# mightypirate1/DRL-Tetris

Hardware: AMD Instinct MI355X
Metric: env-steps/sec at 64k parallel 20x10 boards (higher is better)
Workload: dtype u32

## Files before the change

### drl-tetris_amd/csrc/tetris_aql.h

```cpp
#pragma once
#include <hsa/hsa.h>
#include <hsa/hsa_ext_amd.h>
#include <dlfcn.h>
#include <atomic>
#include <immintrin.h>

namespace aql {

struct Kernel { uint64_t object = 0; uint32_t kernarg = 0, group = 0, priv = 0; bool ok = false; };

struct Queues {
    hsa_queue_t* q[CHAIN_STREAMS] = {};
    char* kernarg[CHAIN_STREAMS] = {};
    uint32_t slot_bytes = 0;
    std::atomic<uint64_t> issued[CHAIN_STREAMS];
    hsa_signal_t gate[CHAIN_STREAMS][2] = {};
    hsa_signal_t done[CHAIN_STREAMS] = {};
    hsa_signal_t first{};
    bool ok = false;
    uint32_t xcd_base[CHAIN_STREAMS] = {};
    bool affine_ok = false, calibrated = false;
};
struct Device {
    int hip_device = -1;
    bool tried = false, ok = false;
    hsa_agent_t gpu{}, cpu{};
    hsa_amd_memory_pool_t dev_pool{};
    uint64_t ts_freq = 0;
    std::vector<hsa_executable_t> exes;
    Kernel chain1, chain1_affine, duo, duo_affine, blocker, xcc_probe;
    std::vector<std::vector<char>> images;
    Queues qs;
    std::string why;
};

constexpr int SLOTS = 4096;
constexpr uint32_t QUEUE_PACKETS = 1024;

static std::mutex g_mutex;
static std::vector<Device*> g_devices;

struct FindCtx { Device* d; uint32_t want_bdf; uint32_t want_domain; bool found_gpu = false, found_cpu = false; };

static hsa_status_t on_agent(hsa_agent_t a, void* p) {
    FindCtx* c = (FindCtx*)p;
    hsa_device_type_t t;
    if (hsa_agent_get_info(a, HSA_AGENT_INFO_DEVICE, &t) != HSA_STATUS_SUCCESS) return HSA_STATUS_SUCCESS;
    if (t == HSA_DEVICE_TYPE_CPU && !c->found_cpu) { c->d->cpu = a; c->found_cpu = true; }
    if (t == HSA_DEVICE_TYPE_GPU && !c->found_gpu) {
        uint32_t bdf = 0, domain = 0;
        (void)hsa_agent_get_info(a, (hsa_agent_info_t)HSA_AMD_AGENT_INFO_BDFID, &bdf);
        (void)hsa_agent_get_info(a, (hsa_agent_info_t)HSA_AMD_AGENT_INFO_DOMAIN, &domain);
        if ((bdf & 0xFFFFu) == c->want_bdf && domain == c->want_domain) { c->d->gpu = a; c->found_gpu = true; }
    }
    return HSA_STATUS_SUCCESS;
}
static hsa_status_t on_gpu_pool(hsa_amd_memory_pool_t p, void* out) {
    Device* d = (Device*)out;
    hsa_amd_segment_t seg;
    uint32_t flags = 0;
    bool alloc = false;
    if (hsa_amd_memory_pool_get_info(p, HSA_AMD_MEMORY_POOL_INFO_SEGMENT, &seg) != HSA_STATUS_SUCCESS || seg != HSA_AMD_SEGMENT_GLOBAL) return HSA_STATUS_SUCCESS;
    (void)hsa_amd_memory_pool_get_info(p, HSA_AMD_MEMORY_POOL_INFO_GLOBAL_FLAGS, &flags);
    (void)hsa_amd_memory_pool_get_info(p, HSA_AMD_MEMORY_POOL_INFO_RUNTIME_ALLOC_ALLOWED, &alloc);
    if (alloc && (flags & HSA_AMD_MEMORY_POOL_GLOBAL_FLAG_COARSE_GRAINED) && d->dev_pool.handle == 0) d->dev_pool = p;
    return HSA_STATUS_SUCCESS;
}
struct SymCtx { Device* d; };
static hsa_status_t on_symbol(hsa_executable_t, hsa_agent_t, hsa_executable_symbol_t s, void* p) {
    Device* d = ((SymCtx*)p)->d;
    hsa_symbol_kind_t kind;
    if (hsa_executable_symbol_get_info(s, HSA_EXECUTABLE_SYMBOL_INFO_TYPE, &kind) != HSA_STATUS_SUCCESS || kind != HSA_SYMBOL_KIND_KERNEL) return HSA_STATUS_SUCCESS;
    uint32_t len = 0;
    (void)hsa_executable_symbol_get_info(s, HSA_EXECUTABLE_SYMBOL_INFO_NAME_LENGTH, &len);
    std::string name(len, '\0');
    (void)hsa_executable_symbol_get_info(s, HSA_EXECUTABLE_SYMBOL_INFO_NAME, &name[0]);
    Kernel* k = nullptr;
    if (name.rfind("_Z7k_chainILi1EEvN2te5KArgsE", 0) == 0) k = &d->chain1;
    else if (name.rfind("_Z5k_duoILi6ELb1ELb0EEvN2te5KArgsE", 0) == 0) k = &d->duo;
    else if (name.rfind("_Z9k_blockerPKjy", 0) == 0) k = &d->blocker;
    else if (name.rfind("_Z14k_chain_affineILi1EEvN2te5KArgsE", 0) == 0) k = &d->chain1_affine;
    else if (name.rfind("tetris_k_xcc_probe", 0) == 0) k = &d->xcc_probe;
    else if (name.rfind("_Z12k_duo_affineN2te5KArgsE", 0) == 0) k = &d->duo_affine;
    if (!k) return HSA_STATUS_SUCCESS;
    bool ok = hsa_executable_symbol_get_info(s, HSA_EXECUTABLE_SYMBOL_INFO_KERNEL_OBJECT, &k->object) == HSA_STATUS_SUCCESS;
    ok = ok && hsa_executable_symbol_get_info(s, HSA_EXECUTABLE_SYMBOL_INFO_KERNEL_KERNARG_SEGMENT_SIZE, &k->kernarg) == HSA_STATUS_SUCCESS;
    ok = ok && hsa_executable_symbol_get_info(s, HSA_EXECUTABLE_SYMBOL_INFO_KERNEL_GROUP_SEGMENT_SIZE, &k->group) == HSA_STATUS_SUCCESS;
    ok = ok && hsa_executable_symbol_get_info(s, HSA_EXECUTABLE_SYMBOL_INFO_KERNEL_PRIVATE_SEGMENT_SIZE, &k->priv) == HSA_STATUS_SUCCESS;
    k->ok = ok && k->object != 0;
    return HSA_STATUS_SUCCESS;
}

static bool own_code_objects(std::vector<std::vector<char>>& out, std::string& why) {
    Dl_info info;
    if (!dladdr((const void*)&own_code_objects, &info) || !info.dli_fname) { why = "dladdr failed"; return false; }
    FILE* f = fopen(info.dli_fname, "rb");
    if (!f) { why = std::string("cannot read ") + info.dli_fname; return false; }
    std::vector<char> file;
    fseek(f, 0, SEEK_END);
    const long len = ftell(f);
    fseek(f, 0, SEEK_SET);
    if (len <= 0) { fclose(f); why = "empty library file"; return false; }
    file.resize((size_t)len);
    const size_t got = fread(file.data(), 1, file.size(), f);
    fclose(f);
    if (got != file.size()) { why = "short read of the library file"; return false; }
    static const char magic[] = "__CLANG_OFFLOAD_BUNDLE__";
    const size_t mlen = sizeof magic - 1;
    for (size_t at = 0; at + mlen + 8 <= file.size(); ) {
        const void* hit = memmem(file.data() + at, file.size() - at, magic, mlen);
        if (!hit) break;
        const size_t base = (size_t)((const char*)hit - file.data());
        at = base + mlen;
        uint64_t n = 0;
        memcpy(&n, file.data() + base + mlen, 8);
        size_t o = base + mlen + 8;
        if (n == 0 || n > 64) continue;
        for (uint64_t e = 0; e < n; e++) {
            if (o + 24 > file.size()) break;
            uint64_t off, size, idlen;
            memcpy(&off, file.data() + o, 8); memcpy(&size, file.data() + o + 8, 8); memcpy(&idlen, file.data() + o + 16, 8);
            o += 24;
            if (idlen > 256 || o + idlen > file.size()) break;
            const std::string id(file.data() + o, (size_t)idlen);
            o += (size_t)idlen;
            if (id.find("amdgcn-amd-amdhsa") != std::string::npos && id.find("gfx950") != std::string::npos && size > 0 &&
                base + off + size <= file.size())
                out.emplace_back(file.data() + base + off, file.data() + base + off + size);
        }
    }
    if (out.empty()) { why = "no gfx950 code object found in the library's fat binary"; return false; }
    return true;
}

static Device* device_for(int hip_device) {
    std::lock_guard<std::mutex> lock(g_mutex);
    for (Device* d : g_devices) if (d->hip_device == hip_device) return d;
    Device* d = new Device();
    d->hip_device = hip_device;
    d->tried = true;
    g_devices.push_back(d);
    auto bad = [&](const std::string& w) { d->why = w; d->ok = false; return d; };
    {
        const char* tools[] = {getenv("ROCP_TOOL_LIBRARIES"), getenv("HSA_TOOLS_LIB"), getenv("LD_PRELOAD")};
        for (const char* t : tools)
            if (t && (strstr(t, "rocprofiler") || strstr(t, "roctracer") || strstr(t, "rocprof")) && !getenv("TETRIS_DIRECT_UNDER_TOOLS"))
                return bad("a profiling tool intercepts the HSA queues");
    }
    hipDeviceProp_t prop;
    if (hipGetDeviceProperties(&prop, hip_device) != hipSuccess) return bad("hipGetDeviceProperties failed");
    if (hsa_init() != HSA_STATUS_SUCCESS) return bad("hsa_init failed");
    FindCtx fc{d, (uint32_t)(((uint32_t)prop.pciBusID << 8) | ((uint32_t)prop.pciDeviceID << 3)), (uint32_t)prop.pciDomainID};
    (void)hsa_iterate_agents(on_agent, &fc);
    if (!fc.found_gpu || !fc.found_cpu) return bad("no HSA agent with the HIP device's PCI address");
    (void)hsa_amd_agent_iterate_memory_pools(d->gpu, on_gpu_pool, d);
    if (d->dev_pool.handle == 0) return bad("no coarse-grained device memory pool");
    (void)hsa_system_get_info(HSA_SYSTEM_INFO_TIMESTAMP_FREQUENCY, &d->ts_freq);
    if (!d->ts_freq) return bad("no timestamp frequency");
    std::string why;
    if (!own_code_objects(d->images, why)) return bad(why);
    for (auto& img : d->images) {
        hsa_code_object_reader_t reader;
        hsa_executable_t exe;
        if (hsa_code_object_reader_create_from_memory(img.data(), img.size(), &reader) != HSA_STATUS_SUCCESS) continue;
        if (hsa_executable_create_alt(HSA_PROFILE_FULL, HSA_DEFAULT_FLOAT_ROUNDING_MODE_DEFAULT, nullptr, &exe) != HSA_STATUS_SUCCESS) continue;
        if (hsa_executable_load_agent_code_object(exe, d->gpu, reader, nullptr, nullptr) != HSA_STATUS_SUCCESS ||
            hsa_executable_freeze(exe, nullptr) != HSA_STATUS_SUCCESS) { (void)hsa_executable_destroy(exe); continue; }
        d->exes.push_back(exe);
        SymCtx sc{d};
        (void)hsa_executable_iterate_agent_symbols(exe, d->gpu, on_symbol, &sc);
    }
    if (!d->chain1.ok || !d->duo.ok) return bad("the chained kernels were not found in the loaded code objects");
    if (d->chain1.priv || d->duo.priv) return bad("the chained kernels use scratch memory");
    const uint32_t explicit_bytes = (uint32_t)((sizeof(KArgs) + 7) & ~(size_t)7);
    if (d->chain1.kernarg < explicit_bytes || d->duo.kernarg < explicit_bytes || d->chain1.kernarg > 1024 || d->duo.kernarg > 1024)
        return bad("unexpected kernel-argument segment size");
    d->ok = true;
    return d;
}

static void destroy_queues(Queues& qs) {
    for (int k = 0; k < CHAIN_STREAMS; k++) {
        if (qs.q[k]) (void)hsa_queue_destroy(qs.q[k]);
        if (qs.kernarg[k]) (void)hsa_amd_memory_pool_free(qs.kernarg[k]);
        for (int s = 0; s < 2; s++) if (qs.gate[k][s].handle) (void)hsa_signal_destroy(qs.gate[k][s]);
        if (qs.done[k].handle) (void)hsa_signal_destroy(qs.done[k]);
    }
    if (qs.first.handle) (void)hsa_signal_destroy(qs.first);
    for (int k = 0; k < CHAIN_STREAMS; k++) { qs.q[k] = nullptr; qs.kernarg[k] = nullptr; qs.done[k] = hsa_signal_t{}; qs.gate[k][0] = qs.gate[k][1] = hsa_signal_t{}; }
    qs.first = hsa_signal_t{}; qs.ok = false; qs.affine_ok = false; qs.calibrated = false;
}

static bool make_queues(Device* d, std::string& why) {
    std::lock_guard<std::mutex> lock(g_mutex);
    Queues& qs = d->qs;
    const int depth = CHAIN_STREAMS;
    if (qs.ok) return true;
    for (int k = 0; k < CHAIN_STREAMS; k++) qs.issued[k].store(0);
    qs.slot_bytes = ((std::max(d->chain1.kernarg, d->duo.kernarg) + 63u) & ~63u) + 64u;
    for (int k = 0; k < depth; k++) {
        if (hsa_queue_create(d->gpu, QUEUE_PACKETS, HSA_QUEUE_TYPE_MULTI, nullptr, nullptr, UINT32_MAX, UINT32_MAX, &qs.q[k]) != HSA_STATUS_SUCCESS) { why = "hsa_queue_create failed"; destroy_queues(qs); return false; }
        (void)hsa_amd_profiling_set_profiler_enabled(qs.q[k], 1);
        if (hsa_amd_memory_pool_allocate(d->dev_pool, (size_t)SLOTS * qs.slot_bytes + 4096, 0, (void**)&qs.kernarg[k]) != HSA_STATUS_SUCCESS ||
            hsa_amd_agents_allow_access(1, &d->cpu, nullptr, qs.kernarg[k]) != HSA_STATUS_SUCCESS) { why = "no host-visible device memory for the kernel arguments"; destroy_queues(qs); return false; }
        for (int s = 0; s < 2; s++)
            if (hsa_signal_create(0, 0, nullptr, &qs.gate[k][s]) != HSA_STATUS_SUCCESS) { why = "hsa_signal_create failed"; destroy_queues(qs); return false; }
        if (hsa_signal_create(0, 0, nullptr, &qs.done[k]) != HSA_STATUS_SUCCESS) { why = "hsa_signal_create failed"; destroy_queues(qs); return false; }
    }
    if (hsa_signal_create(0, 0, nullptr, &qs.first) != HSA_STATUS_SUCCESS) { why = "hsa_signal_create failed"; destroy_queues(qs); return false; }
    qs.ok = true;
    return true;
}

static void fill_hidden(char* slot, uint32_t explicit_bytes, uint32_t slot_bytes, uint32_t blocks, uint32_t group) {
    char* h = slot + explicit_bytes;
    const uint32_t room = slot_bytes - explicit_bytes;
    if (room < 72) return;
    const uint32_t bc[3] = {blocks, 1u, 1u};
    const uint16_t gs[3] = {(uint16_t)group, 1, 1};
    const uint16_t dims = 1;
    memcpy(h + 0, bc, 12);
    memcpy(h + 12, gs, 6);
    memcpy(h + 64, &dims, 2);
}

static inline bool wait_signal(hsa_signal_t s) {
    for (int round = 0; round < 4000; round++)
        if (hsa_signal_wait_scacquire(s, HSA_SIGNAL_CONDITION_LT, 1, 2000000, HSA_WAIT_STATE_ACTIVE) < 1) return true;
    return hsa_signal_wait_scacquire(s, HSA_SIGNAL_CONDITION_LT, 1, UINT64_MAX, HSA_WAIT_STATE_BLOCKED) < 1;
}

struct Pending {
    uint64_t written[CHAIN_STREAMS] = {}, rung[CHAIN_STREAMS] = {};
    bool wrote[CHAIN_STREAMS] = {};
    char* last_slot = nullptr;
};
static inline void ring(Queues& qs, Pending& pd) {
    if (pd.last_slot) { _mm_sfence(); (void)*(volatile uint32_t*)pd.last_slot; pd.last_slot = nullptr; }
    for (int k = 0; k < CHAIN_STREAMS; k++)
        if (pd.wrote[k] && pd.written[k] != pd.rung[k]) {
            hsa_signal_store_screlease(qs.q[k]->doorbell_signal, (hsa_signal_value_t)(pd.written[k] - 1));
            pd.rung[k] = pd.written[k];
        }
}
static inline char* claim_packet(Queues& qs, Pending& pd, int k) {
    hsa_queue_t* q = qs.q[k];
    const uint64_t idx = hsa_queue_add_write_index_relaxed(q, 1);
    while (idx - hsa_queue_load_read_index_scacquire(q) >= q->size) ring(qs, pd);
    pd.written[k] = idx + 1; pd.wrote[k] = true;
    return (char*)q->base_address + (idx & (q->size - 1)) * 64;
}
static inline void write_dispatch(Queues& qs, Pending& pd, int k, const Kernel& kern, const void* args, size_t arg_bytes, uint32_t blocks,
                                  int acquire, int release, hsa_signal_t signal) {
    char* slot = qs.kernarg[k] + (size_t)(qs.issued[k].fetch_add(1) % SLOTS) * qs.slot_bytes;
    memcpy(slot, args, arg_bytes);
    fill_hidden(slot, (uint32_t)((arg_bytes + 7) & ~(size_t)7), qs.slot_bytes, blocks, 64);
    pd.last_slot = slot;
    char* p = claim_packet(qs, pd, k);
    hsa_kernel_dispatch_packet_t* d = (hsa_kernel_dispatch_packet_t*)p;
    d->setup = 1 << HSA_KERNEL_DISPATCH_PACKET_SETUP_DIMENSIONS;
    d->workgroup_size_x = 64; d->workgroup_size_y = 1; d->workgroup_size_z = 1; d->reserved0 = 0;
    d->grid_size_x = blocks * 64u; d->grid_size_y = 1; d->grid_size_z = 1;
    d->private_segment_size = kern.priv; d->group_segment_size = kern.group;
    d->kernel_object = kern.object; d->kernarg_address = slot; d->reserved2 = 0; d->completion_signal = signal;
    const uint16_t header = (uint16_t)((HSA_PACKET_TYPE_KERNEL_DISPATCH << HSA_PACKET_HEADER_TYPE) | (1 << HSA_PACKET_HEADER_BARRIER) |
                                       (acquire << HSA_PACKET_HEADER_SCACQUIRE_FENCE_SCOPE) | (release << HSA_PACKET_HEADER_SCRELEASE_FENCE_SCOPE));
    __atomic_store_n((uint16_t*)p, header, __ATOMIC_RELEASE);
}
static inline void write_barrier(Queues& qs, Pending& pd, int k, hsa_signal_t signal, int scope = HSA_FENCE_SCOPE_SYSTEM) {
    char* p = claim_packet(qs, pd, k);
    memset(p + 2, 0, 62);
    ((hsa_barrier_and_packet_t*)p)->completion_signal = signal;
    const uint16_t header = (uint16_t)((HSA_PACKET_TYPE_BARRIER_AND << HSA_PACKET_HEADER_TYPE) | (1 << HSA_PACKET_HEADER_BARRIER) |
                                       (scope << HSA_PACKET_HEADER_SCACQUIRE_FENCE_SCOPE) | (scope << HSA_PACKET_HEADER_SCRELEASE_FENCE_SCOPE));
    __atomic_store_n((uint16_t*)p, header, __ATOMIC_RELEASE);
}

static void calibrate_affine(Device* d) {
    std::lock_guard<std::mutex> lock(g_mutex);
    Queues& qs = d->qs;
    if (!qs.ok || qs.calibrated) return;
    qs.calibrated = true;
    { const char* e = getenv("TETRIS_AFFINE"); if (e && e[0] == '0') return; }
    if (!d->xcc_probe.ok || !d->chain1_affine.ok || d->xcc_probe.priv || d->chain1_affine.priv || (d->duo_affine.ok && d->duo_affine.priv)) return;
    constexpr uint32_t BLOCKS = 1024;
    const size_t words = (size_t)2 * CHAIN_STREAMS * BLOCKS;
    uint32_t* out = nullptr;
    if (hsa_amd_memory_pool_allocate(d->dev_pool, words * 4, 0, (void**)&out) != HSA_STATUS_SUCCESS) return;
    std::vector<uint32_t> host(words, 0xFFu);
    bool ok = hsa_memory_copy(out, host.data(), words * 4) == HSA_STATUS_SUCCESS;
    for (int rep = 0; rep < 2 && ok; rep++) {
        Pending pd;
        for (int k = 0; k < CHAIN_STREAMS; k++) {
            struct { uint32_t* out; } args = {out + ((size_t)rep * CHAIN_STREAMS + k) * BLOCKS};
            hsa_signal_store_relaxed(qs.done[k], 1);
            write_dispatch(qs, pd, k, d->xcc_probe, &args, sizeof args, BLOCKS, HSA_FENCE_SCOPE_SYSTEM, HSA_FENCE_SCOPE_SYSTEM, qs.done[k]);
        }
        ring(qs, pd);
        for (int k = 0; k < CHAIN_STREAMS; k++) ok = wait_signal(qs.done[k]) && ok;
    }
    ok = ok && hsa_memory_copy(host.data(), out, words * 4) == HSA_STATUS_SUCCESS;
    (void)hsa_amd_memory_pool_free(out);
    if (!ok) return;
    for (int k = 0; k < CHAIN_STREAMS; k++) {
        const uint32_t* a = &host[(size_t)k * BLOCKS];
        const uint32_t* b = &host[((size_t)CHAIN_STREAMS + k) * BLOCKS];
        if (a[0] > 7u || a[0] != b[0]) return;
        for (uint32_t i = 0; i < BLOCKS; i++)
            if (a[i] != ((a[0] + i) & 7u) || b[i] != a[i]) return;
        qs.xcd_base[k] = a[0];
    }
    qs.affine_ok = true;
}

static inline void quiesce(Queues& qs) {
    if (!qs.ok) return;
    Pending pd;
    for (int k = 0; k < CHAIN_STREAMS; k++)
        if (qs.q[k]) { hsa_signal_store_relaxed(qs.done[k], 1); write_barrier(qs, pd, k, qs.done[k]); }
    ring(qs, pd);
    for (int k = 0; k < CHAIN_STREAMS; k++)
        if (qs.q[k]) (void)wait_signal(qs.done[k]);
}

}
```

### drl-tetris_amd/csrc/tetris_engine.h

```cpp
#pragma once
#include "tetris_layout.h"
#include "tetris_tables.h"

#if defined(__clang__)
#define TE_UNROLL _Pragma("unroll")
#else
#define TE_UNROLL _Pragma("GCC unroll 8")
#endif

namespace te {

TE_HD int ctz32(uint32_t v) { return __builtin_ctz(v); }
TE_HD int clz32(uint32_t v) { return __builtin_clz(v); }
#if defined(__HIP_DEVICE_COMPILE__)
TE_HD uint32_t ld_stream(const uint32_t* p) { return __builtin_nontemporal_load(p); }
TE_HD void st_stream(uint32_t* p, uint32_t v) { __builtin_nontemporal_store(v, p); }
#else
TE_HD uint32_t ld_stream(const uint32_t* p) { return *p; }
TE_HD void st_stream(uint32_t* p, uint32_t v) { *p = v; }
#endif

#if defined(TE_PATH_COUNTERS) && !defined(__HIPCC__)
enum PathCounter { PC_KICK = 0, PC_KICK_2ND, PC_KICK_3RD, PC_KICK_FAILED, PC_KICK_DOWN, PC_DROP_EXACT, PC_RT_OFF_SPAWN,
                   PC_GARBAGE_ROW, PC_GARBAGE_LIFT2, PC_DEATH_GARBAGE, PC_DEATH_SPAWN, PC_TIMER_LOCK, PC_KEY_KICK, PC_KEY_KICK_FAILED,
                   PC_UNDO_SIMPLE, PC_UNDO_FULL, PC_UNDO_MISPREDICT, PC_NCOUNTERS };
extern unsigned long long te_path_count[PC_NCOUNTERS];
#define TE_COUNT(i) (te_path_count[i]++)
#else
#define TE_COUNT(i) do {} while (0)
#endif

enum MemMode : int { MEM_STREAM = 0, MEM_AGENT = 1, MEM_AFFINE = 2 };
#if defined(__HIP_DEVICE_COMPILE__)
TE_HD uint32_t ld_agent(const uint32_t* p) { return __hip_atomic_load(p, __ATOMIC_RELAXED, __HIP_MEMORY_SCOPE_AGENT); }
TE_HD void st_agent(uint32_t* p, uint32_t v) { __hip_atomic_store(p, v, __ATOMIC_RELAXED, __HIP_MEMORY_SCOPE_AGENT); }
#else
TE_HD uint32_t ld_agent(const uint32_t* p) { return *p; }
TE_HD void st_agent(uint32_t* p, uint32_t v) { *p = v; }
#endif
#if defined(__HIP_DEVICE_COMPILE__)
TE_HD __amdgpu_buffer_rsrc_t te_rsrc(const void* base) {
    return __builtin_amdgcn_make_buffer_rsrc(const_cast<void*>(base), (short)0, -1, 0x00020000);
}
constexpr int TE_AUX_NT = 2, TE_AUX_SC1 = 16;
TE_HD uint32_t ldw(const uint32_t* base, uint32_t o, size_t word_off, int mem = MEM_STREAM) {
    const __amdgpu_buffer_rsrc_t r = te_rsrc(base);
    if (mem == MEM_AGENT || mem == MEM_AFFINE) return __builtin_amdgcn_raw_buffer_load_b32(r, (int)o, (int)(uint32_t)(word_off * 4u), TE_AUX_SC1);
    return __builtin_amdgcn_raw_buffer_load_b32(r, (int)o, (int)(uint32_t)(word_off * 4u), TE_AUX_NT);
}
TE_HD void stw(uint32_t* base, uint32_t o, size_t word_off, uint32_t v, int mem = MEM_STREAM) {
    const __amdgpu_buffer_rsrc_t r = te_rsrc(base);
    if (mem == MEM_AGENT) __builtin_amdgcn_raw_buffer_store_b32(v, r, (int)o, (int)(uint32_t)(word_off * 4u), TE_AUX_SC1);
    else if (mem == MEM_AFFINE) __builtin_amdgcn_raw_buffer_store_b32(v, r, (int)o, (int)(uint32_t)(word_off * 4u), 0);
    else __builtin_amdgcn_raw_buffer_store_b32(v, r, (int)o, (int)(uint32_t)(word_off * 4u), TE_AUX_NT);
}
#else
TE_HD uint32_t ldw(const uint32_t* base, uint32_t o, size_t word_off, int mem = MEM_STREAM) {
    const uint32_t* p = (const uint32_t*)((const char*)(base + word_off) + o);
    return mem != MEM_STREAM ? ld_agent(p) : ld_stream(p);
}
TE_HD void stw(uint32_t* base, uint32_t o, size_t word_off, uint32_t v, int mem = MEM_STREAM) {
    uint32_t* p = (uint32_t*)((char*)(base + word_off) + o);
    if (mem != MEM_STREAM) st_agent(p, v); else st_stream(p, v);
}
#endif
#if defined(__HIP_DEVICE_COMPILE__)
TE_HD void add_word(uint32_t* p, uint32_t v) { (void)__hip_atomic_fetch_add(p, v, __ATOMIC_RELAXED, __HIP_MEMORY_SCOPE_AGENT); }
#else
TE_HD void add_word(uint32_t* p, uint32_t v) { *p += v; }
#endif
#if defined(__HIP_DEVICE_COMPILE__)
TE_HD uint32_t mul24(uint32_t a, uint32_t b) { return __umul24(a, b); }
#else
TE_HD uint32_t mul24(uint32_t a, uint32_t b) { return a * b; }
#endif
TE_HD int imin(int a, int b) { return a < b ? a : b; }
TE_HD int imax(int a, int b) { return a > b ? a : b; }
TE_HD uint32_t f2u(float f) { union { float f; uint32_t u; } v; v.f = f; return v.u; }
TE_HD float u2f(uint32_t u) { union { float f; uint32_t u; } v; v.u = u; return v.f; }

constexpr uint16_t SHAPE_ROWS[7][4] = {
    {0x2260, 0x0710, 0x3220, 0x4700}, {0x2230, 0x1700, 0x6220, 0x0740}, {0x2640, 0x0630, 0x1320, 0x6300},
    {0x2310, 0x3600, 0x4620, 0x0360}, {0x2222, 0x0f00, 0x4444, 0x00f0}, {0x0720, 0x2320, 0x2700, 0x2620},
    {0x0660, 0x0660, 0x0660, 0x0660},
};
TE_HD int spawn_rot(int kind) { return (int)((0x0977u >> (2 * (kind & 7))) & 3u); }
TE_HD int shape_value(int kind) { return (int)((0x06127534u >> (4 * (kind & 7))) & 15u); }

constexpr uint32_t make_shape(int kind, int rot) {
    uint32_t rows = SHAPE_ROWS[kind][rot];
    uint32_t nibs = 0;
    for (int gy = 0; gy < 4; gy++) {
        uint32_t rown = (rows >> (4 * (3 - gy))) & 0xF;
        for (int gx = 0; gx < 4; gx++)
            if ((rown >> gx) & 1) nibs |= 1u << (4 * gx + gy);
    }
    int minc = 3, maxc = 0;
    for (int gx = 0; gx < 4; gx++)
        if ((nibs >> (4 * gx)) & 0xF) { if (gx < minc) minc = gx; if (gx > maxc) maxc = gx; }
    return nibs | ((uint32_t)minc << 16) | ((uint32_t)maxc << 18);
}
constexpr uint32_t make_drop_word(uint32_t nibs) {
    uint32_t w = 0;
    for (int gx = 0; gx < 4; gx++) {
        uint32_t n = (nibs >> (4 * gx)) & 0xF;
        int bottom = -1;
        for (int gy = 0; gy < 4; gy++)
            if ((n >> gy) & 1) bottom = gy;
        w |= (uint32_t)(bottom < 0 ? 0x7F : 0x40 - (bottom + 1)) << (8 * gx);
    }
    return w;
}
constexpr int SHAPE_WORDS = 64;
struct ShapeTable { uint32_t s[SHAPE_WORDS]; };
constexpr ShapeTable make_shape_table() {
    ShapeTable t{};
    for (int k = 0; k < 7; k++)
        for (int r = 0; r < 4; r++) {
            t.s[k * 4 + r] = make_shape(k, r);
            t.s[32 + k * 4 + r] = make_drop_word(t.s[k * 4 + r] & 0xFFFFu);
        }
    for (int r = 0; r < 4; r++) { t.s[28 + r] = 0; t.s[60 + r] = 0x7F7F7F7Fu; }
    return t;
}
constexpr ShapeTable SHAPES = make_shape_table();

struct Ctx {
    const uint32_t* shapes;
    const uint8_t* table;
    const uint64_t* start;
    const double* combo_pow;
    uint32_t n_draws;
    uint32_t margin;
    int H;
    uint32_t floor_bits;
    bool tint;
    bool queue;
};

constexpr int ERR_FIFO = 1;
constexpr int ERR_STREAM = 2;

struct Raw8 { uint32_t lo, hi; };
struct Player {
    uint32_t col[NCOL];
    uint32_t tint[3][NCOL];
    int kind, rot, x, y, next;
    int dead, lock_armed, reward;
    int inc_count, combo_count, line_count, qlen;
    int q_overflow;
    int32_t time_ms, drop_delay, drop_time, speedup_time, lock_time;
    int32_t combo_start, combo_time, min_remaining;
    uint32_t combo_remaining;
    float incoming;
    uint32_t piece_draws, hole_draws;
    uint32_t pgroup;
    uint32_t lines_sent, lines_cleared, lines_blocked, max_combo, lines_seen, garbage_cleared;
    int32_t qcount[FIFO_CAP];
    int32_t qdelay[FIFO_CAP];
    int q_loaded;
    Raw8 pf_raw;
    int pf_ok;
};

struct ResetPrefetch { uint32_t seed16; uint64_t word; int ok; };

template <int P>
struct Game {
    Player pl[P];
    uint32_t seed16;
    int round_over, last_winner;
    uint32_t flags;
    uint32_t episode;
    uint32_t steps;
    uint32_t add_lines, add_sent;
    uint32_t status;
    uint32_t draw0, draw1;
};

TE_HD void load_player(const uint32_t* s, uint32_t o, size_t ws, Player& q, bool tint, bool queue = true, int mem = MEM_STREAM) {
    for (int c = 0; c < NCOL; c++) q.col[c] = ldw(s, o, (size_t)(W_COL0 + c) * ws, mem);
    if (tint)
        for (int k = 0; k < 3; k++)
            for (int c = 0; c < NCOL; c++) q.tint[k][c] = ldw(s, o, (size_t)(W_TINT0 + 10 * k + c) * ws, mem);
    uint32_t w = ldw(s, o, (size_t)W_PIECE * ws, mem);
    q.kind = w & 7; q.rot = (w >> 3) & 3; q.x = (int)((w >> 5) & 15) - 4; q.y = (w >> 9) & 31;
    q.next = (w >> 14) & 7; q.dead = (w >> 17) & 1; q.lock_armed = (w >> 18) & 1; q.reward = (w >> 19) & 255;
    w = ldw(s, o, (size_t)W_MISC * ws, mem);
    q.inc_count = w & 255; q.combo_count = (w >> 8) & 255; q.line_count = (w >> 16) & 255;
    q.qlen = (w >> 24) & 15; q.q_overflow = (w >> 28) & 3;
    if (!queue) { q.inc_count = 0; q.qlen = 0; q.q_overflow = 0; }
    q.time_ms = (int32_t)ldw(s, o, (size_t)W_TIME * ws, mem);
    w = ldw(s, o, (size_t)W_DROPCOMBO * ws, mem);
    q.drop_delay = w & 0xFFFF; q.combo_remaining = w >> 16;
    q.drop_time = (int32_t)ldw(s, o, (size_t)W_DROP_TIME * ws, mem);
    q.speedup_time = (int32_t)ldw(s, o, (size_t)W_SPEEDUP_TIME * ws, mem);
    q.lock_time = (int32_t)ldw(s, o, (size_t)W_LOCK_TIME * ws, mem);
    q.combo_start = (int32_t)ldw(s, o, (size_t)W_COMBO_START * ws, mem);
    q.combo_time = (int32_t)ldw(s, o, (size_t)W_COMBO_TIME * ws, mem);
    q.incoming = queue ? u2f(ldw(s, o, (size_t)W_INCOMING * ws, mem)) : 0.0f;
    q.min_remaining = queue ? (int32_t)ldw(s, o, (size_t)W_MIN_REMAINING * ws, mem) : 1000;
    q.piece_draws = ldw(s, o, (size_t)W_PIECE_DRAWS * ws, mem);
    q.hole_draws = queue ? ldw(s, o, (size_t)W_HOLE_DRAWS * ws, mem) : 0u;
    q.pgroup = ldw(s, o, (size_t)W_PIECE_GROUP * ws, mem);
    w = ldw(s, o, (size_t)W_STATS0 * ws, mem); q.lines_sent = w & 0xFFFF; q.lines_cleared = w >> 16;
    w = ldw(s, o, (size_t)W_STATS1 * ws, mem); q.lines_blocked = w & 0xFFFF; q.max_combo = w >> 16;
    w = ldw(s, o, (size_t)W_STATS2 * ws, mem); q.lines_seen = w & 0xFFFF; q.garbage_cleared = w >> 16;
    q.q_loaded = queue && q.qlen > 0;
    q.pf_ok = 0; q.pf_raw.lo = 0; q.pf_raw.hi = 0;
    if (queue)
        for (int i = 0; i < FIFO_CAP; i++) { q.qcount[i] = 0; q.qdelay[i] = 0; }
    if (q.q_loaded) {
        for (int i = 0; i < FIFO_CAP / 2; i++) {
            uint32_t cw = ldw(s, o, (size_t)(W_FIFO_COUNT0 + i) * ws, mem);
            q.qcount[2 * i] = (int16_t)(cw & 0xFFFF);
            q.qcount[2 * i + 1] = (int16_t)(cw >> 16);
        }
        for (int i = 0; i < FIFO_CAP; i++) q.qdelay[i] = (int32_t)ldw(s, o, (size_t)(W_FIFO_DELAY0 + i) * ws, mem);
    }
}

template <int P>
TE_HD void load_game_words(const Ref& gr, Game<P>& g, bool counters = false, int mem = MEM_STREAM) {
    uint32_t meta = ldw(gr.s, gr.o, (size_t)G_META * gr.ws, mem);
    g.seed16 = meta & 0xFFFFu;
    g.round_over = (meta >> 16) & 1;
    g.last_winner = (int)((meta >> 17) & 0xF) - 1;
    g.flags = (meta >> 21) & 7u;
    g.episode = ldw(gr.s, gr.o, (size_t)G_EPISODE * gr.ws, mem);
    g.steps = counters ? ldw(gr.s, gr.o, (size_t)G_STEPS * gr.ws, mem) : 0u;
    g.add_lines = 0; g.add_sent = 0;
    g.status = 0;
}

template <int P>
TE_HD void load_game(const Geo& geo_in, size_t slot, Game<P>& g, bool tint = false, bool queue = true, bool counters = false, int mem = MEM_STREAM) {
    Geo geo = geo_in;
    geo.P = P;
    load_game_words<P>(game_ref(geo, slot), g, counters, mem);
    TE_UNROLL
    for (int p = 0; p < P; p++) {
        const Ref r = board_ref(geo, p, slot);
        load_player(r.s, r.o, r.ws, g.pl[p], tint, queue, mem);
    }
}

TE_HD void store_player(uint32_t* s, uint32_t o, size_t ws, const Player& q, bool tint, bool queue = true, int mem = MEM_STREAM) {
    for (int c = 0; c < NCOL; c++) stw(s, o, (size_t)(W_COL0 + c) * ws, q.col[c], mem);
    if (tint)
        for (int k = 0; k < 3; k++)
            for (int c = 0; c < NCOL; c++) stw(s, o, (size_t)(W_TINT0 + 10 * k + c) * ws, q.tint[k][c], mem);
    stw(s, o, (size_t)W_PIECE * ws, (uint32_t)q.kind | ((uint32_t)q.rot << 3) | ((uint32_t)(q.x + 4) << 5) | ((uint32_t)q.y << 9) |
                              ((uint32_t)q.next << 14) | ((uint32_t)q.dead << 17) | ((uint32_t)q.lock_armed << 18) |
                              ((uint32_t)(q.reward & 255) << 19), mem);
    stw(s, o, (size_t)W_MISC * ws, (uint32_t)(q.inc_count & 255) | ((uint32_t)(q.combo_count & 255) << 8) |
                             ((uint32_t)(q.line_count & 255) << 16) | ((uint32_t)q.qlen << 24) | ((uint32_t)q.q_overflow << 28), mem);
    stw(s, o, (size_t)W_TIME * ws, (uint32_t)q.time_ms, mem);
    stw(s, o, (size_t)W_DROPCOMBO * ws, ((uint32_t)q.drop_delay & 0xFFFF) | (q.combo_remaining << 16), mem);
    stw(s, o, (size_t)W_DROP_TIME * ws, (uint32_t)q.drop_time, mem);
    stw(s, o, (size_t)W_SPEEDUP_TIME * ws, (uint32_t)q.speedup_time, mem);
    stw(s, o, (size_t)W_LOCK_TIME * ws, (uint32_t)q.lock_time, mem);
    stw(s, o, (size_t)W_COMBO_START * ws, (uint32_t)q.combo_start, mem);
    stw(s, o, (size_t)W_COMBO_TIME * ws, (uint32_t)q.combo_time, mem);
    if (queue) stw(s, o, (size_t)W_INCOMING * ws, f2u(q.incoming), mem);
    stw(s, o, (size_t)W_MIN_REMAINING * ws, (uint32_t)q.min_remaining, mem);
    stw(s, o, (size_t)W_PIECE_DRAWS * ws, q.piece_draws, mem);
    if (queue) stw(s, o, (size_t)W_HOLE_DRAWS * ws, q.hole_draws, mem);
    stw(s, o, (size_t)W_PIECE_GROUP * ws, q.pgroup, mem);
    stw(s, o, (size_t)W_STATS0 * ws, (q.lines_sent & 0xFFFF) | (q.lines_cleared << 16), mem);
    stw(s, o, (size_t)W_STATS1 * ws, (q.lines_blocked & 0xFFFF) | (q.max_combo << 16), mem);
    stw(s, o, (size_t)W_STATS2 * ws, (q.lines_seen & 0xFFFF) | (q.garbage_cleared << 16), mem);
    if (queue && (q.q_loaded || q.qlen > 0)) {
        for (int i = 0; i < FIFO_CAP / 2; i++)
            stw(s, o, (size_t)(W_FIFO_COUNT0 + i) * ws, ((uint32_t)q.qcount[2 * i] & 0xFFFF) | ((uint32_t)q.qcount[2 * i + 1] << 16), mem);
        for (int i = 0; i < FIFO_CAP; i++) stw(s, o, (size_t)(W_FIFO_DELAY0 + i) * ws, (uint32_t)q.qdelay[i], mem);
    }
}

template <int P>
TE_HD void store_game_words(const Ref& gr, const Game<P>& g, bool counters = false, int mem = MEM_STREAM) {
    stw(gr.s, gr.o, (size_t)G_META * gr.ws, g.seed16 | ((uint32_t)g.round_over << 16) | ((uint32_t)(g.last_winner + 1) << 17) | (g.flags << 21), mem);
    stw(gr.s, gr.o, (size_t)G_EPISODE * gr.ws, g.episode, mem);
    if (counters) stw(gr.s, gr.o, (size_t)G_STEPS * gr.ws, g.steps, mem);
    if (g.add_lines) add_word(&word_at(gr, G_LINES), g.add_lines);
    if (g.add_sent) add_word(&word_at(gr, G_SENT), g.add_sent);
}

template <int P>
TE_HD void store_game(const Geo& geo_in, size_t slot, const Game<P>& g, bool tint = false, bool queue = true, bool counters = false, int mem = MEM_STREAM) {
    Geo geo = geo_in;
    geo.P = P;
    store_game_words<P>(game_ref(geo, slot), g, counters, mem);
    TE_UNROLL
    for (int p = 0; p < P; p++) {
        const Ref r = board_ref(geo, p, slot);
        store_player(r.s, r.o, r.ws, g.pl[p], tint, queue, mem);
    }
}


TE_HD uint32_t shape_of(const Ctx& cx, int kind, int rot) { return cx.shapes[(kind << 2) | rot]; }

TE_HD uint64_t band_window(const Ctx& cx, const Player& q, int y) {
    uint32_t lo = 0xFFu, hi = 0xFFFF0000u;
    for (int c = 0; c < 6; c++) lo |= ((uint32_t)((int32_t)(q.col[c] | cx.floor_bits) >> y) & 0xFu) << (4 * c + 8);
    for (int c = 6; c < NCOL; c++) hi |= ((uint32_t)((int32_t)(q.col[c] | cx.floor_bits) >> y) & 0xFu) << (4 * (c - 6));
    return ((uint64_t)hi << 32) | lo;
}

TE_HD bool fits_band(uint64_t band, uint32_t shape, int x) {
    unsigned xs = (unsigned)(x + 2);
    if (xs > 12u) return false;
    return (((uint64_t)(shape & 0xFFFFu) << (4 * xs)) & band) == 0;
}

TE_HD bool fits_at(const Ctx& cx, const Player& q, uint32_t shape, int x, int y) {
    return fits_band(band_window(cx, q, y), shape, x);
}

TE_HD bool fits_spawn_col(const Ctx& cx, const Player& q, uint32_t shape, int y) {
    constexpr int X0 = (NCOL - 4) / 2;
    uint32_t hit = 0;
    TE_UNROLL
    for (int gx = 0; gx < 4; gx++) hit |= (q.col[X0 + gx] | cx.floor_bits) & (((shape >> (4 * gx)) & 0xFu) << y);
    return hit == 0;
}

TE_HD uint32_t col_at(const Player& q, int i) {
    uint32_t a0 = (i & 1) ? q.col[1] : q.col[0];
    uint32_t a1 = (i & 1) ? q.col[3] : q.col[2];
    uint32_t a2 = (i & 1) ? q.col[5] : q.col[4];
    uint32_t a3 = (i & 1) ? q.col[7] : q.col[6];
    uint32_t a4 = (i & 1) ? q.col[9] : q.col[8];
    uint32_t b0 = (i & 2) ? a1 : a0;
    uint32_t b1 = (i & 2) ? a3 : a2;
    uint32_t d0 = (i & 4) ? b1 : b0;
    return (i & 8) ? a4 : d0;
}

TE_HD int drop_distance(const Ctx& cx, const Player& q, uint32_t shape) {
    int dist = 64;
    for (int gx = 0; gx < 4; gx++) {
        uint32_t nib = (shape >> (4 * gx)) & 0xFu;
        if (nib) {
            int top = q.y + ctz32(nib);
            int bottom = q.y + (31 - clz32(nib));
            uint32_t below = (col_at(q, q.x + gx) | cx.floor_bits) >> (top + 1);
            int first = below ? ctz32(below) + top + 1 : 32;
            dist = imin(dist, imax(0, first - bottom - 1));
        }
    }
    return dist == 64 ? 0 : dist;
}

TE_HD int drop_distance_bytes(const Ctx& cx, const Player& q, uint32_t shape, uint32_t drop_word) {
    uint32_t d[NCOL];
    for (int c = 0; c < NCOL; c++) d[c] = (uint32_t)ctz32((q.col[c] | cx.floor_bits) >> q.y);
    const uint32_t w0 = (d[0] << 16) | (d[1] << 24);
    const uint32_t w1 = d[2] | (d[3] << 8) | (d[4] << 16) | (d[5] << 24);
    const uint32_t w2 = d[6] | (d[7] << 8) | (d[8] << 16) | (d[9] << 24);
    const unsigned xs = (unsigned)(q.x + 2);
    const bool hi2 = (xs & 8u) != 0, hi1 = (xs & 4u) != 0;
    const uint32_t lo = hi2 ? (hi1 ? 0u : w2) : (hi1 ? w1 : w0);
    const uint32_t hi = hi2 ? 0u : (hi1 ? w2 : w1);
#if defined(__HIP_DEVICE_COMPILE__)
    const uint32_t under = __builtin_amdgcn_alignbyte(hi, lo, xs & 3u);
#else
    const uint32_t under = (uint32_t)((((uint64_t)hi << 32) | lo) >> (8 * (xs & 3u)));
#endif
    const uint32_t sum = under + drop_word;
    const uint32_t b0 = sum & 0xFFu, b1 = (sum >> 8) & 0xFFu, b2 = (sum >> 16) & 0xFFu, b3 = sum >> 24;
    const uint32_t m01 = b0 < b1 ? b0 : b1, m23 = b2 < b3 ? b2 : b3;
    const uint32_t m = m01 < m23 ? m01 : m23;
    if (m - 0x40u > 0x3Eu) { TE_COUNT(PC_DROP_EXACT); return drop_distance(cx, q, shape); }
    return (int)(m - 0x40u);
}

TE_HD void stamp(const Ctx& cx, Player& q, uint32_t shape) {
    unsigned xs = (unsigned)(q.x + 2);
    if (xs > 12u) return;
    uint64_t placed = (uint64_t)(shape & 0xFFFFu) << (4 * xs);
    for (int c = 0; c < NCOL; c++) {
        const uint32_t cells = ((uint32_t)(placed >> (4 * c + 8)) & 0xFu) << q.y;
        q.col[c] |= cells;
        if (cx.tint)
            for (int k = 0; k < 3; k++) q.tint[k][c] = (q.tint[k][c] & ~cells) | (((q.kind >> k) & 1) ? cells : 0u);
    }
}

TE_HD int clear_rows(const Ctx& cx, Player& q) {
    uint32_t range = (~0u << q.y) & ~cx.floor_bits;
    int cleared = 0;
    for (;;) {
        uint32_t full = range;
        for (int c = 0; c < NCOL; c++) full &= q.col[c];
        if (!full) break;
        int r = 31 - clz32(full);
        uint32_t above = (1u << r) - 1u;
        uint32_t keep = ~((above << 1) | 1u);
        if (cx.tint) {
            uint32_t garbage = 0;
            for (int c = 0; c < NCOL; c++) garbage |= q.col[c] & q.tint[0][c] & q.tint[1][c] & q.tint[2][c];
            if ((garbage >> r) & 1u) q.garbage_cleared = (q.garbage_cleared + 1u) & 0xFFFFu;
            for (int k = 0; k < 3; k++)
                for (int c = 0; c < NCOL; c++) q.tint[k][c] = (q.tint[k][c] & keep) | ((q.tint[k][c] & above) << 1);
        }
        for (int c = 0; c < NCOL; c++) q.col[c] = (q.col[c] & keep) | ((q.col[c] & above) << 1);
        cleared++;
    }
    return cleared;
}

TE_HD uint32_t table_byte(const Ctx& cx, uint32_t seed16, uint32_t draw, uint32_t& status) {
    if (draw + cx.margin >= cx.n_draws) {
        status |= ST_NEED_EXTEND;
        if (draw >= cx.n_draws) { status |= ST_STREAM_EXHAUSTED; draw = cx.n_draws - 1; }
    }
    uint32_t chunk = draw / (uint32_t)CHUNK;
    uint32_t r = draw - mul24(chunk, (uint32_t)CHUNK);
    return cx.table[mul24((chunk << 16) + seed16, (uint32_t)CHUNK) + r];
}

TE_HD Raw8 table_group_raw(const Ctx& cx, uint32_t seed16, uint32_t draw, uint32_t& status) {
    if (draw + 8u + cx.margin >= cx.n_draws) {
        status |= ST_NEED_EXTEND;
        if (draw + 8u > cx.n_draws) { status |= ST_STREAM_EXHAUSTED; draw = cx.n_draws - 8u; }
    }
    uint32_t chunk = draw / (uint32_t)CHUNK;
    uint32_t r = draw - mul24(chunk, (uint32_t)CHUNK);
    const uint8_t* p = cx.table + (mul24((chunk << 16) + seed16, (uint32_t)CHUNK) + r);
    Raw8 v;
#if defined(__HIP_DEVICE_COMPILE__)
    const uint2 w = *reinterpret_cast<const uint2*>(p);
    v.lo = w.x; v.hi = w.y;
#else
    v.lo = 0; v.hi = 0;
    for (int k = 0; k < 4; k++) { v.lo |= (uint32_t)p[k] << (8 * k); v.hi |= (uint32_t)p[4 + k] << (8 * k); }
#endif
    return v;
}
TE_HD uint32_t pack_group(Raw8 v) {
    const uint32_t a = v.lo & 0x0F0F0F0Fu, b = v.hi & 0x0F0F0F0Fu;
    uint32_t lo = (a | (a >> 4)) & 0x00FF00FFu; lo = (lo | (lo >> 8)) & 0x0000FFFFu;
    uint32_t hi = (b | (b >> 4)) & 0x00FF00FFu; hi = (hi | (hi >> 8)) & 0x0000FFFFu;
    return lo | (hi << 16);
}

TE_HD void prefetch_next(const Ctx& cx, Player& q, uint32_t seed16, uint32_t& status) {
    q.pf_ok = 0;
    if ((q.piece_draws & 7u) == 7u) {
// ... 833 lines not shown
```

### drl-tetris_amd/csrc/tetris_hip.hip

```cpp
#include <hip/hip_runtime.h>
#include <hip/hip_ext.h>

#include <math.h>
#include <stdio.h>
#include <stdlib.h>
#include <string.h>

#include <algorithm>
#include <atomic>
#include <mutex>
#include <thread>
#include <new>
#include <chrono>
#include <string>
#include <vector>

#include "tetris_kernels.h"

using namespace te;


#include "tetris_game_kernel.h"

constexpr int CHAIN_LANES = 64;
constexpr int CHAIN_STREAMS = 3;
template <int P, bool AFFINE>
__device__ __forceinline__ void chain_body(const KArgs& a) {
    __shared__ __attribute__((aligned(16))) uint32_t s_shapes[SHAPE_WORDS];
    const int lane = threadIdx.x;
    if (a.steps < 0) { chain_census(a, lane == 0); return; }
    constexpr int CMEM = AFFINE ? MEM_AFFINE : MEM_AGENT;
    int wave = blockIdx.x;
    uint32_t xcc = 0;
    const auto report_xcc = [&]() { if (AFFINE && blockIdx.x == 0 && lane == 0) st_flag(a.status + F_XCC0 + (a.xcd_slot & 3u), 0x100u | xcc); };
    if (AFFINE) {
        asm volatile("s_getreg_b32 %0, hwreg(HW_REG_XCC_ID)" : "=s"(xcc));
        xcc &= 0xFu;
        if (xcc != ((a.xcd_base + blockIdx.x) & 7u)) {
            if (lane == 0) st_flag(a.status + F_PLACE, 1u);
            report_xcc();
            return;
        }
        wave = (int)((blockIdx.x & ~7u) | xcc);
        if (wave * CHAIN_LANES >= a.n) { report_xcc(); return; }
    }
    const int i = wave * CHAIN_LANES + lane;
    const bool active = lane < CHAIN_LANES && i < a.n;
    LaneCounters cnt = {0, 0, 0, 0};
    const uint32_t shape_word = d_shape_table.s[lane];
    Game<P> g;
    if (active) policy_draw(a, (uint32_t)i, a.first_step, g.draw0, g.draw1);
    const uint32_t d0 = g.draw0, d1 = g.draw1;
    int stride = a.n_stride;
    asm volatile("" : "+s"(stride));
    const uint32_t seen = chain_poll(a, (uint32_t)wave);
    if (seen == a.epoch - 1u) {
        Geo geo = geo_of(a);
        geo.stride = (size_t)stride;
        if (active) { load_game<P>(geo, (size_t)i, g, false, P > 1, true, CMEM); g.draw0 = d0; g.draw1 = d1; }
        s_shapes[lane] = shape_word;
        __builtin_amdgcn_wave_barrier();
        if (active) game_run<P, M_ROLLOUT, false, CMEM>(a, i, s_shapes, g, cnt);
        asm volatile("s_waitcnt vmcnt(0)" ::: "memory");
        if (lane == 0) {
            if (AFFINE) st_xcd(a.chain + (size_t)wave * CHAIN_STRIDE, a.epoch);
            else st_agent(a.chain + (size_t)wave * CHAIN_STRIDE, a.epoch);
        }
    } else if (!(seen & CHAIN_ABANDONED)) {
        chain_give_up(a, (uint32_t)wave, lane == 0);
    }
    report_xcc();
}
template <int P>
__global__ __launch_bounds__(64) void k_chain(KArgs a) { chain_body<P, false>(a); }
template <int P>
__global__ __launch_bounds__(64) void k_chain_affine(KArgs a) { chain_body<P, true>(a); }
template __global__ void k_chain_affine<1>(KArgs);
extern "C" __global__ void tetris_k_xcc_probe(uint32_t* out) {
    if (threadIdx.x == 0) {
        uint32_t xcc;
        asm volatile("s_getreg_b32 %0, hwreg(HW_REG_XCC_ID)" : "=s"(xcc));
        out[blockIdx.x] = xcc & 0xFu;
    }
}

__global__ void k_blocker(const uint32_t* go, unsigned long long ticks) {
    const unsigned long long t0 = __builtin_amdgcn_s_memrealtime();
    while (__builtin_amdgcn_s_memrealtime() - t0 < ticks) {
        if (go && __hip_atomic_load(go, __ATOMIC_RELAXED, __HIP_MEMORY_SCOPE_SYSTEM)) break;
        __builtin_amdgcn_s_sleep(32);
    }
}

__global__ void k_clock_probe(unsigned long long ticks, unsigned long long* out) {
    const unsigned long long r0 = __builtin_amdgcn_s_memrealtime(), c0 = __builtin_amdgcn_s_memtime();
    unsigned long long r1 = r0;
    while (r1 - r0 < ticks) { __builtin_amdgcn_s_sleep(4); r1 = __builtin_amdgcn_s_memrealtime(); }
    const unsigned long long c1 = __builtin_amdgcn_s_memtime();
    if (threadIdx.x == 0) { out[0] = c1 - c0; out[1] = r1 - r0; }
}

__global__ __launch_bounds__(256) void k_totals(Geo geo, unsigned long long* out ) {
    unsigned long long v[4] = {0, 0, 0, 0};
    for (int i = blockIdx.x * blockDim.x + threadIdx.x; i < (int)geo.n_games; i += gridDim.x * blockDim.x) {
        unsigned long long t[4];
        totals_of_game(geo, i, t);
        v[0] += t[0]; v[1] += t[1]; v[2] += t[2]; v[3] += t[3];
    }
    for (int k = 0; k < 4; k++) {
        for (int off = 32; off > 0; off >>= 1) v[k] += __shfl_down(v[k], off);
        if ((threadIdx.x & 63) == 0 && v[k]) atomicAdd(&out[k], v[k]);
    }
}

#define TE_OBS_BUILD(a, row, sl, i, COL, qx, qy, qnext, qkind, qinc, qcombo, qrem)                                              \
    do {                                                                                                                        \
        uint32_t col_[NCOL];                                                                                                    \
        TE_UNROLL                                                                                                               \
        for (int c = 0; c < NCOL; c++) col_[c] = COL(c);                                                                        \
        for (int yp = 0; yp < (a).H / 2; yp++) {                                                                                \
            uint32_t lo[NCOL], hi[NCOL];                                                   \
            TE_UNROLL                                                                                                           \
            for (int c = 0; c < NCOL; c++) { lo[c] = col_[c] & 1u; hi[c] = (col_[c] >> 1) & 1u; col_[c] >>= 2; }                \
            (row)[5 * yp + 0] = lo[0] | (lo[1] << 8) | (lo[2] << 16) | (lo[3] << 24);                                           \
            (row)[5 * yp + 1] = lo[4] | (lo[5] << 8) | (lo[6] << 16) | (lo[7] << 24);                                           \
            (row)[5 * yp + 2] = lo[8] | (lo[9] << 8) | (hi[0] << 16) | (hi[1] << 24);                                           \
            (row)[5 * yp + 3] = hi[2] | (hi[3] << 8) | (hi[4] << 16) | (hi[5] << 24);                                           \
            (row)[5 * yp + 4] = hi[6] | (hi[7] << 8) | (hi[8] << 16) | (hi[9] << 24);                                           \
        }                                                                                                                       \
                             \
        const uint32_t x_ = (uint32_t)(qx) & 0xFFu, y_ = (uint32_t)(qy) & 31u, next_ = (uint32_t)(qnext) & 7u;                  \
        uint32_t t_ = (((uint32_t)(qrem) & 0xFFFFu) + 50u) & 0xFFFFu;  \
        if (t_ > 25000u) t_ = 25000u;                                                                                           \
        uint32_t* v_ = (uint32_t*)((a).obs_vector + ((size_t)(sl) * (a).n + (i)) * 12);                                         \
        const uint64_t hot_ = next_ < 7u ? (1ull << (8 * next_)) : 0ull;                                       \
        v_[0] = x_ | (y_ << 8) | (((uint32_t)(qinc) & 255u) << 16) | ((t_ / 100u) << 24);                                       \
        v_[1] = ((uint32_t)(qcombo) & 255u) | ((uint32_t)(hot_ & 0xFFFFFFu) << 8);                                              \
        v_[2] = (uint32_t)(hot_ >> 24);                                                                                         \
        (a).obs_piece[(size_t)(sl) * (a).n + (i)] = (uint8_t)((uint32_t)(qkind) & 7u);                                          \
    } while (0)
__device__ __forceinline__ void obs_build(const KArgs& a, uint32_t* row, int sl, int i, uint32_t c0, uint32_t c1, uint32_t c2, uint32_t c3, uint32_t c4,
                                          uint32_t c5, uint32_t c6, uint32_t c7, uint32_t c8, uint32_t c9, int qx, int qy, int qnext, int qkind,
                                          int inc_count, int combo_count, uint32_t combo_remaining) {
    const uint32_t cols[NCOL] = {c0, c1, c2, c3, c4, c5, c6, c7, c8, c9};
#define TE_OBS_COL(c) cols[c]
    TE_OBS_BUILD(a, row, sl, i, TE_OBS_COL, qx, qy, qnext, qkind, inc_count, combo_count, combo_remaining);
#undef TE_OBS_COL
}
__device__ __forceinline__ void obs_stream(const KArgs& a, const uint32_t* rows, int sl, int first, int nb, int lane) {
    const int nw = a.H * NCOL / 4;
    uint32_t* dst = (uint32_t*)(a.obs_visual + ((size_t)sl * a.n + first) * (size_t)(a.H * NCOL));
    const uint32_t words = (uint32_t)nb * (uint32_t)nw;
    typedef uint32_t u32x4 __attribute__((ext_vector_type(4)));
    if (((((uintptr_t)dst) | ((uintptr_t)rows)) & 15u) == 0) {
        const uint32_t whole = words & ~3u;
        for (uint32_t k = 4u * (uint32_t)lane; k < whole; k += 4u * 64u)
            __builtin_nontemporal_store(*reinterpret_cast<const u32x4*>(rows + k), reinterpret_cast<u32x4*>(dst + k));
        if ((uint32_t)lane < words - whole) dst[whole + lane] = rows[whole + lane];
    } else
        for (uint32_t k = (uint32_t)lane; k < words; k += 64u) dst[k] = rows[k];
}

template <int P>
__device__ __forceinline__ void observe_emit(const KArgs& a, const Game<P>& g, int first, int lane, bool active, uint32_t* tile) {
    const int pitch = a.H * NCOL / 4, i = first + lane;
    const int nb = (a.n - first < 64) ? a.n - first : 64;
    const int me = active ? safe_player(a.next_player, i, P) : 0;
    TE_UNROLL
    for (int sl = 0; sl < P; sl++) {
        if (active) {
            const bool sel = P > 1 && (sl == 0 ? me == 1 : me == 0);
            const Player& q0 = g.pl[0];
            const Player& q1 = g.pl[P - 1];
            uint32_t* row = tile + (size_t)lane * pitch;
#define TE_OBS_COL(c) (sel ? q1.col[c] : q0.col[c])
            TE_OBS_BUILD(a, row, sl, i, TE_OBS_COL, sel ? q1.x : q0.x, sel ? q1.y : q0.y, sel ? q1.next : q0.next, sel ? q1.kind : q0.kind,
                         sel ? q1.inc_count : q0.inc_count, sel ? q1.combo_count : q0.combo_count, sel ? q1.combo_remaining : q0.combo_remaining);
#undef TE_OBS_COL
        }
        __syncthreads();
        obs_stream(a, tile, sl, first, nb, lane);
        __syncthreads();
    }
}

template <int MODE, bool CHAIN, bool OBS, bool AFFINE>
__device__ __forceinline__ void duo_body(const KArgs& a) {
    __shared__ __attribute__((aligned(16))) uint32_t s_shapes_all[4][SHAPE_WORDS];
    extern __shared__ __attribute__((aligned(16))) uint32_t s_duo_tile[];
    uint32_t* s_shapes = s_shapes_all[threadIdx.x >> 6];
    const uint32_t shape_word = d_shape_table.s[threadIdx.x & 63];
    const int lane = threadIdx.x & 63, side = lane >> 5;
    int wave = (blockIdx.x * blockDim.x + threadIdx.x) >> 6;
    constexpr bool ROLL = MODE == M_ROLLOUT, AUTO = MODE == M_STEP_RT_AUTO;
    constexpr int MEM = CHAIN ? (AFFINE ? MEM_AFFINE : MEM_AGENT) : MEM_STREAM;
    if (CHAIN && a.steps < 0) { chain_census(a, lane == 0); return; }
    uint32_t xcc = 0;
    const auto report_xcc = [&]() { if (AFFINE && blockIdx.x == 0 && lane == 0) st_flag(a.status + F_XCC0 + (a.xcd_slot & 3u), 0x100u | xcc); };
    if (AFFINE) {
        asm volatile("s_getreg_b32 %0, hwreg(HW_REG_XCC_ID)" : "=s"(xcc));
        xcc &= 0xFu;
        if (xcc != ((a.xcd_base + blockIdx.x) & 7u)) {
            if (lane == 0) st_flag(a.status + F_PLACE, 1u);
            report_xcc();
            return;
        }
        wave = (int)((blockIdx.x & ~7u) | xcc);
        if (wave * 32 >= a.n) { report_xcc(); return; }
    }
    const int gi = wave * 32 + (lane & 31);
    const bool active = gi < a.n;
    Geo geo = geo_of(a);
    geo.P = 2;
    const Ref gr = game_ref(geo, (size_t)gi);
    const Ref br = {geo.state, (uint32_t)((size_t)side * geo.stride + (size_t)gi) * 4u, 2 * geo.stride};
    Game<1> g;
    Player& q = g.pl[0];
    uint32_t pd0 = 0, pd1 = 0;
    if (CHAIN) {
        if (active) policy_draw(a, (uint32_t)gi, a.first_step, pd0, pd1);
        if (!chain_wait(a, (uint32_t)wave, lane == 0)) { report_xcc(); return; }
    }
    if (active) {
        load_game_words<1>(gr, g, ROLL, MEM);
        load_player(br.s, br.o, br.ws, q, false, true, MEM);
        if (CHAIN) { g.draw0 = pd0; g.draw1 = pd1; }
        else if (ROLL) policy_draw(a, (uint32_t)gi, a.first_step, g.draw0, g.draw1);
        else { g.draw0 = a.rot[gi]; g.draw1 = (uint32_t)a.trans[gi] | ((a.player ? (uint32_t)a.player[gi] : 0u) << 8); }
    }
    s_shapes[lane] = shape_word;
// ... 449 lines not shown
struct Tables {
    int device = -1;
    uint8_t map[8] = {0};
    int only_sz = 0;
    int refs = 0;
    uint32_t* d_mt = nullptr;
    float* d_w = nullptr;
    uint64_t* d_start = nullptr;
    double* d_pow = nullptr;
    uint8_t* d_table = nullptr;
    int n_chunks = 0, cap_chunks = 0;
    std::vector<uint8_t*> retired;
};
static const size_t CHUNK_BYTES = (size_t)65536 * CHUNK;
static std::mutex g_tab_mutex;
static std::vector<Tables*> g_tables;

static int tables_extend(Tables* t, hipStream_t stream) {
    if (t->n_chunks >= MAX_CHUNKS) return fail(TETRIS_E_STREAM, "RNG tables: MAX_CHUNKS reached");
    if (t->n_chunks == t->cap_chunks) {
        int cap = t->cap_chunks ? t->cap_chunks * 2 : 2;
        if (cap > MAX_CHUNKS) cap = MAX_CHUNKS;
        uint8_t* d = nullptr;
        HIP_TRY(hipMalloc((void**)&d, CHUNK_BYTES * cap));
        if (t->n_chunks) HIP_TRY(hipMemcpyAsync(d, t->d_table, CHUNK_BYTES * t->n_chunks, hipMemcpyDeviceToDevice, stream));
        if (t->d_table) t->retired.push_back(t->d_table);
        t->d_table = d;
        t->cap_chunks = cap;
    }
    MapArg m;
    memcpy(m.m, t->map, 8);
    hipLaunchKernelGGL(k_gen_chunk, dim3(256), dim3(256), 0, stream, t->d_mt, t->d_w, t->d_table + CHUNK_BYTES * t->n_chunks,
                       t->d_start, t->n_chunks, m, t->only_sz);
    HIP_TRY(hipGetLastError());
    HIP_TRY(hipStreamSynchronize(stream));
    t->n_chunks++;
    return TETRIS_OK;
}

static void tables_free(Tables* t) {
    (void)hipFree(t->d_mt); (void)hipFree(t->d_w); (void)hipFree(t->d_start); (void)hipFree(t->d_pow);
    (void)hipFree(t->d_table);
    for (uint8_t* c : t->retired) (void)hipFree(c);
    delete t;
}

static int tables_build(Tables* t, hipStream_t stream);

static int tables_acquire(Tables** out, int device, const uint8_t map[7], hipStream_t stream) {
    std::lock_guard<std::mutex> lock(g_tab_mutex);
    for (Tables* t : g_tables)
        if (t->device == device && memcmp(t->map, map, 7) == 0) { t->refs++; *out = t; return TETRIS_OK; }
    Tables* t = new (std::nothrow) Tables();
    if (!t) return fail(TETRIS_E_HIP, "out of host memory");
    t->device = device;
    memcpy(t->map, map, 7);
    t->only_sz = 1;
    for (int i = 0; i < 7; i++) if (map[i] != 2 && map[i] != 3) t->only_sz = 0;
    int rc = tables_build(t, stream);
    if (rc) { std::string keep = g_err; tables_free(t); return fail(rc, keep); }
    t->refs = 1;
    g_tables.push_back(t);
    *out = t;
    return TETRIS_OK;
}

static int tables_build(Tables* t, hipStream_t stream) {
    HIP_TRY(hipMalloc((void**)&t->d_mt, (size_t)624 * 65536 * 4));
    HIP_TRY(hipMalloc((void**)&t->d_w, (size_t)7 * 65536 * 4));
    HIP_TRY(hipMalloc((void**)&t->d_start, 65536 * sizeof(uint64_t)));
    HIP_TRY(hipMalloc((void**)&t->d_pow, 256 * sizeof(double)));
    double powtab[256];
    for (int c = 0; c < 256; c++) powtab[c] = pow((double)c, 1.4 + (double)c * 0.01);
    HIP_TRY(hipMemcpyAsync(t->d_pow, powtab, sizeof powtab, hipMemcpyHostToDevice, stream));
    hipLaunchKernelGGL(k_gen_seed, dim3(256), dim3(256), 0, stream, t->d_mt);
    HIP_TRY(hipGetLastError());
    HIP_TRY(hipStreamSynchronize(stream));
    for (int c = 0; c < 2; c++) {
        int rc = tables_extend(t, stream);
        if (rc) return rc;
    }
    return TETRIS_OK;
}

static void tables_release(Tables* t) {
    std::lock_guard<std::mutex> lock(g_tab_mutex);
    if (--t->refs > 0) return;
    for (size_t i = 0; i < g_tables.size(); i++)
        if (g_tables[i] == t) { g_tables.erase(g_tables.begin() + i); break; }
    tables_free(t);
}

struct Stage {
    void* h = nullptr;
    void* d = nullptr;
    size_t cap = 0;
    int ensure(size_t bytes) {
        if (bytes <= cap) return TETRIS_OK;
        size_t want = bytes < 4096 ? 4096 : bytes + bytes / 2;
        if (h) (void)hipHostFree(h);
        if (d) (void)hipFree(d);
        h = d = nullptr; cap = 0;
        HIP_TRY(hipHostMalloc(&h, want, hipHostMallocDefault));
        HIP_TRY(hipMalloc(&d, want));
        cap = want;
        return TETRIS_OK;
    }
    void release() {
        if (h) (void)hipHostFree(h);
        if (d) (void)hipFree(d);
        h = d = nullptr; cap = 0;
    }
};
constexpr int STAGES = 6;

constexpr int GATE_GROUP = 120;
#include "tetris_aql.h"

struct RolloutCall {
    uint32_t epoch0 = 0;
    uint64_t first_step = 0;
    int steps_per_launch = 0;
    uint32_t policy_seed = 0;
    int ms = 0;
    int launches = 0;
    bool chained = false;
};

struct tetris_batch {
    int device = 0, N = 0, P = 0, H = 0;
    int stride = 0;
    hipStream_t stream = nullptr;
    hipEvent_t ev0 = nullptr, ev1 = nullptr;
    uint32_t* d_state = nullptr;
    uint32_t* d_gstate = nullptr;
    uint32_t* flags = nullptr;
    unsigned long long* d_counters = nullptr;
    unsigned long long* h_counters = nullptr;
    Tables* tab = nullptr;
    uint32_t margin = 2 * (2 * GATE_GROUP + 2) + 16;
    uint32_t game_offset = 0;
    int split = 0, side = 0;
    int tint = 0, nw = NWORDS;
    int use_duo = 1;
    uint32_t* d_shadow = nullptr;
    hipStream_t own_stream = nullptr;
    hipStream_t chain_stream[CHAIN_STREAMS] = {};
    hipEvent_t chain_ev[CHAIN_STREAMS + 1] = {};
    hipEvent_t worker_gate_ev[CHAIN_STREAMS][2] = {};
    uint32_t* d_chain = nullptr;
    uint32_t chain_epoch = 0;
    int use_chain = 1;
    int use_graph = 0;
    long long chain_capacity = -1;
    int chain_depth = 0;
    bool chain_pending = false;
    uint32_t chain_spin_limit = CHAIN_SPIN_LIMIT;
    RolloutCall chain_call;
    bool chain_fell_back = false;
    uint32_t* h_chain = nullptr;
    hipStream_t stall_stream = nullptr;
    int direct_min = 16;
    bool last_direct = false;
    bool direct_used = false;
    int use_affine = 1;
    bool last_affine = false;
    uint32_t xcd_skew = 0;
    int affine_failures = 0;
    bool home_async = false;
    bool busy = true;
    hipEvent_t gate_ev[2] = {nullptr, nullptr};
    int gate_count = 0;
    int gate_slot = 0;
    int gate_pending[2] = {0, 0};
    Stage stage[STAGES];
    Stage recover_idx;
    uint8_t* d_plan_slabs = nullptr;
    size_t plan_slab_cap = 0;
    int32_t* d_iota = nullptr;
    uint32_t* d_plan_status = nullptr;
    int32_t* d_policy_scores = nullptr;
};

static Geo geo_of_batch(tetris_batch* b) {
    Geo g = {b->d_state, b->d_gstate, (size_t)b->N, b->P, b->nw, (size_t)b->stride};
    return g;
}

static KArgs base_args(tetris_batch* b, int n, const int32_t* d_idx) {
    KArgs a;
    memset(&a, 0, sizeof a);
    a.state = b->d_state; a.gstate = b->d_gstate; a.status = b->flags;
    {
        std::lock_guard<std::mutex> lock(g_tab_mutex);
        a.table = b->tab->d_table;
        a.n_draws = (uint32_t)b->tab->n_chunks * CHUNK;
    }
    a.start = b->tab->d_start; a.combo_pow = b->tab->d_pow; a.margin = b->margin;
    a.H = b->H; a.n_games = b->N; a.n_stride = b->stride; a.n_players = b->P; a.nw = b->nw; a.n = n; a.idx = d_idx; a.game_offset = b->game_offset;
    return a;
}

template <int MODE>
static int launch_game(tetris_batch* b, const KArgs& a) {
    dim3 grid((unsigned)((a.n + 255) / 256)), block(256);
    if constexpr (MODE == M_ROLLOUT || MODE == M_STEP_RT || MODE == M_STEP_RT_AUTO) {
        if (b->P == 2 && !b->tint && !a.idx && b->use_duo && (MODE != M_ROLLOUT || a.steps == 1)) {
            hipLaunchKernelGGL((k_duo<MODE>), dim3((unsigned)((a.n + 127) / 128)), block, 0, b->stream, a);
            HIP_TRY(hipGetLastError());
            return TETRIS_OK;
        }
    }
    const bool here = with_shape<1, 2>(b->P, b->tint != 0, [&](auto P, auto TINT) {
        hipLaunchKernelGGL((k_game<P(), MODE, TINT()>), grid, block, 0, b->stream, a);
    });
    if (!here && tetris_launch_game_multi(b->P, b->tint, MODE, grid, block, b->stream, a)) return fail(TETRIS_E_ARG, "no kernel for this player count / mode");
    HIP_TRY(hipGetLastError());
    return TETRIS_OK;
}

static int chain_lanes(const tetris_batch* b) { return b->P == 1 ? CHAIN_LANES : 32; }
static uint32_t chain_waves(const tetris_batch* b) { return (uint32_t)((b->N + chain_lanes(b) - 1) / chain_lanes(b)); }

static const void* chain_kernel(tetris_batch* b, long long* waves) {
    *waves = chain_waves(b);
    return b->P == 1 ? (const void*)k_chain<1> : (const void*)k_duo<M_ROLLOUT, true>;
}
static hipError_t launch_chain_kernel(tetris_batch* b, uint32_t blocks, hipStream_t st, const KArgs& a, hipEvent_t start = nullptr,
                                      hipEvent_t stop = nullptr) {
    if (b->P == 1) hipExtLaunchKernelGGL((k_chain<1>), dim3(blocks), dim3(64), 0, st, start, stop, 0, a);
    else hipExtLaunchKernelGGL((k_duo<M_ROLLOUT, true>), dim3(blocks), dim3(64), 0, st, start, stop, 0, a);
    return hipGetLastError();
}
static bool chain_census_ok(tetris_batch* b, long long waves) {
    uint32_t* d = nullptr;
    if (hipMalloc((void**)&d, 2 * CHAIN_STRIDE * sizeof(uint32_t)) != hipSuccess) return false;
    bool ok = false;
    uint32_t h[2] = {0, 1};
    KArgs a;
    memset(&a, 0, sizeof a);
    a.steps = -1; a.chain = d; a.epoch = (uint32_t)waves; a.chain_spin_limit = 4000;
    if (hipMemsetAsync(d, 0, 2 * CHAIN_STRIDE * sizeof(uint32_t), b->own_stream) == hipSuccess) {
        if (launch_chain_kernel(b, (uint32_t)waves, b->own_stream, a) == hipSuccess && hipMemcpyAsync(&h[0], d, 4, hipMemcpyDeviceToHost, b->own_stream) == hipSuccess &&
            hipMemcpyAsync(&h[1], d + CHAIN_STRIDE, 4, hipMemcpyDeviceToHost, b->own_stream) == hipSuccess &&
            hipStreamSynchronize(b->own_stream) == hipSuccess)
            ok = h[0] == (uint32_t)waves && h[1] == 0;
    }
    (void)hipFree(d);
    return ok;
}

static bool chain_fits(tetris_batch* b) {
    long long waves = 0;
    const void* fn = chain_kernel(b, &waves);
    static const int cap = [] { const char* e = getenv("TETRIS_CHAIN_DEPTH"); const int v = e ? atoi(e) : CHAIN_STREAMS; return v < 1 ? 1 : (v > CHAIN_STREAMS ? CHAIN_STREAMS : v); }();
    if (b->chain_capacity < 0) {
        int per_cu = 0, cus = 0;
        if (hipOccupancyMaxActiveBlocksPerMultiprocessor(&per_cu, fn, 64, 0) != hipSuccess) per_cu = 0;
        if (hipDeviceGetAttribute(&cus, hipDeviceAttributeMultiprocessorCount, b->device) != hipSuccess) cus = 0;
        b->chain_capacity = per_cu > 1 ? (long long)(per_cu - 1) * cus : 0;
        const long long full = (long long)per_cu * cus;
        int want = 0;
        for (int d = cap; d >= 2 && !want; d--)
            if (d * waves <= full) want = d;
        if (want && want * waves > b->chain_capacity && b->stream == b->own_stream && chain_census_ok(b, want * waves)) b->chain_capacity = want * waves;
    }
    b->chain_depth = 0;
    for (int d = cap; d >= 1 && !b->chain_depth; d--)
        if (d * waves <= b->chain_capacity) b->chain_depth = d;
    return b->chain_depth >= (cap == 1 ? 1 : 2);
}

static int service_flags(tetris_batch* b) {
    volatile uint32_t* f = b->flags;
    const uint32_t want = f[F_EXTEND];
    if (want) {
        std::lock_guard<std::mutex> lock(g_tab_mutex);
        if (want >= (uint32_t)b->tab->n_chunks * CHUNK && b->tab->n_chunks < MAX_CHUNKS) {
            int rc = tables_extend(b->tab, b->stream);
            if (rc) return rc;
            b->busy = true;
        }
        f[F_EXTEND] = 0;
    }
    return TETRIS_OK;
}

static hipError_t poll_event(hipEvent_t e, int spins) {
    hipError_t qe = hipErrorNotReady;
    for (int spin = 0; spin < spins && qe == hipErrorNotReady; spin++) qe = hipEventQuery(e);
    return qe == hipErrorNotReady ? hipEventSynchronize(e) : qe;
}

static int gate_launch(tetris_batch* b, int group) {
    if (b->gate_count >= group) {
        const int k = b->gate_slot;
        if (b->gate_pending[k]) {
            HIP_TRY(poll_event(b->gate_ev[k], 2000000));
            b->gate_pending[k] = 0;
        }
        HIP_TRY(hipEventRecord(b->gate_ev[k], b->stream));
        b->gate_pending[k] = 1;
        b->gate_slot = k ^ 1;
        b->gate_count = 0;
    }
    b->gate_count++;
    {
        bool on_chain = false;
        for (hipStream_t st : b->chain_stream) on_chain |= b->stream == st;
        if (!on_chain) b->home_async = true;
    }
    return service_flags(b);
}

static hipError_t drain_stream(hipStream_t st) {
    for (int spin = 0; spin < 20000; spin++) {
        const hipError_t e = hipStreamQuery(st);
        if (e != hipErrorNotReady) return e;
    }
    return hipStreamSynchronize(st);
}

static int finish_call(tetris_batch* b, bool drained = false) {
    if (!b->busy && !b->chain_pending && b->stream == b->own_stream) {
        int rc0 = service_flags(b);
        if (rc0) return rc0;
        if (!b->busy) return TETRIS_OK;
    }
    if (b->chain_pending && !drained)
        for (int k = 0; k < CHAIN_STREAMS; k++) HIP_TRY(drain_stream(b->chain_stream[k]));
    b->chain_pending = false;
    if (!drained) HIP_TRY(drain_stream(b->stream));
    b->home_async = false;
    b->busy = false;
    b->gate_count = 0; b->gate_pending[0] = b->gate_pending[1] = 0;
    volatile uint32_t* f = b->flags;
    int rc = TETRIS_OK;
    const bool misplaced = f[F_PLACE] != 0;
    if (misplaced) {
        const int keep_chain = b->use_chain;
        const bool keep_fell_back = b->chain_fell_back;
        f[F_PLACE] = 0;
        if ((rc = chain_recover(b))) return rc;
        b->use_chain = keep_chain; b->chain_fell_back = keep_fell_back;
        if (++b->affine_failures >= 3) b->use_affine = 0;
    }
    if (f[F_CHAIN] && (rc = chain_recover(b))) return rc;
    if ((rc = service_flags(b))) return rc;
    if (f[F_BADARG]) {
        f[F_BADARG] = 0;
        return fail(TETRIS_E_ARG, "output capacity exceeded (max_lists / max_keys too small)");
    }
    return TETRIS_OK;
}

static int check_batch(tetris_batch* b, bool enqueues = true) {
    if (!b) return fail(TETRIS_E_ARG, "null batch");
    HIP_TRY(hipSetDevice(b->device));
    if (enqueues) b->busy = true;
    return TETRIS_OK;
}

struct HostCall {
    tetris_batch* const b;
    const int32_t* d_idx = nullptr;
    int used = 0, n_out = 0;
    struct Out { const Stage* s; size_t bytes; void* dst; } outs[STAGES];

    int take(size_t bytes, Stage** s) {
        if (used >= STAGES) return fail(TETRIS_E_ARG, "internal: a call takes more than STAGES staging buffers");
        *s = &b->stage[used++];
        return (*s)->ensure(bytes + 16);
    }
    int send(const Stage* s, size_t bytes) {
        b->busy = true;
        HIP_TRY(hipMemcpyAsync(s->d, s->h, bytes, hipMemcpyHostToDevice, b->stream));
        return TETRIS_OK;
    }
    template <class T> int in(const T* src, size_t count, const T** d) {
        *d = nullptr;
        if (!src) { used++; return TETRIS_OK; }
        Stage* s;
        int rc = take(count * sizeof(T), &s);
        if (rc) return rc;
        memcpy(s->h, src, count * sizeof(T));
        *d = (const T*)s->d;
        return send(s, count * sizeof(T));
    }
    int idx(const int32_t* idx, int n) {
        if (n < 0 || (!idx && n > b->N)) return fail(TETRIS_E_ARG, "n out of range");
        for (int i = 0; idx && i < n; i++)
            if (idx[i] < 0 || idx[i] >= b->N) return fail(TETRIS_E_ARG, "game index out of range");
        return in(idx, (size_t)n, &d_idx);
    }
    template <class T> int out(void* dst, size_t count, T** d, const T** h = nullptr) {
        Stage* s;
        int rc = take(count * sizeof(T), &s);
        if (rc) return rc;
        outs[n_out++] = {s, count * sizeof(T), dst};
        *d = (T*)s->d;
        if (h) *h = (const T*)s->h;
        return TETRIS_OK;
    }
    int finish() {
        for (int k = 0; k < n_out; k++) {
            b->busy = true;
            HIP_TRY(hipMemcpyAsync(outs[k].s->h, outs[k].s->d, outs[k].bytes, hipMemcpyDeviceToHost, b->stream));
        }
        int rc = finish_call(b);
        if (rc) return rc;
        for (int k = 0; k < n_out; k++)
            if (outs[k].dst) memcpy(outs[k].dst, outs[k].s->h, outs[k].bytes);
        return TETRIS_OK;
    }
};

static int check_players(const tetris_batch* b, const uint8_t* player, int n) {
    for (int i = 0; player && i < n; i++)
        if (player[i] >= b->P) return fail(TETRIS_E_ARG, "player index out of range");
    return TETRIS_OK;
}

// ... 738 lines not shown
        uint8_t *d_cnt, *d_len, *d_key;
        if ((rc = io.idx(h_idx, m)) || (rc = io.in(player ? player + g0 : nullptr, (size_t)m, &d_player)) ||
            (rc = io.out(nullptr, lanes, &d_cnt, &hc)) || (rc = io.out(nullptr, lanes * L, &d_len, &hl)) ||
            (rc = io.out(nullptr, lanes * L * max_keys, &d_key, &hk))) return rc;
        dim3 grid((unsigned)((lanes + 63) / 64)), block(64);
        with_value<1, 4>(b->P, [&](auto P) {
            hipLaunchKernelGGL(k_actions<P()>, grid, block, 0, b->stream, geo_of_batch(b), m, io.d_idx, d_player, b->H, d_cnt, d_len, d_key,
                               PLAN_LANE_LISTS, max_keys, b->flags);
        });
        if (hipGetLastError() != hipSuccess) return fail(TETRIS_E_HIP, "k_actions launch failed");
        if ((rc = io.finish())) return rc;
        for (int i = 0; i < m; i++) {
            int total = 0;
            bool over = false;
            for (int xi = 0; xi < 10; xi++)
                for (int r = 0; r < 4; r++) {
                    const size_t lane = (size_t)i * 40 + r * 10 + xi;
                    for (int k = 0; k < hc[lane]; k++) {
                        if (total >= max_lists) { over = true; break; }
                        const int len = hl[lane * L + k];
                        lens[(size_t)(g0 + i) * max_lists + total] = (uint8_t)len;
                        memcpy(keys + ((size_t)(g0 + i) * max_lists + total) * max_keys, hk + (lane * L + k) * max_keys, (size_t)len);
                        total++;
                    }
                }
            count[g0 + i] = total;
            if (over) return fail(TETRIS_E_ARG, "more than max_lists key lists for one game");
        }
    }
    return TETRIS_OK;
}

static const int PLAN_CHUNK = 4096;

static int plan_check(tetris_batch* b, const char* what) {
    if (b->split) return fail(TETRIS_E_ARG, std::string(what) + " is not available on split batches");
    return TETRIS_OK;
}

static PlanArgs plan_args(tetris_batch* b, const uint8_t* d_player, const int32_t* d_count, const uint8_t* d_lens, const uint8_t* d_keys,
                          int max_lists, int max_keys, int ms) {
    PlanArgs pa;
    memset(&pa, 0, sizeof pa);
    pa.a = base_args(b, b->N, nullptr);
    pa.a.ms = ms;
    pa.player = d_player; pa.count = d_count; pa.lens = d_lens; pa.keys = d_keys;
    pa.max_lists = max_lists; pa.max_keys = max_keys;
    return pa;
}

static int launch_plan_kernel(tetris_batch* b, int which, dim3 grid, const PlanArgs& pa, int fin) {
    const bool here = with_shape<1, 2>(b->P, b->tint != 0, [&](auto P, auto TINT) { launch_plan<P(), TINT()>(which, grid, b->stream, pa, fin); });
    if (!here && tetris_launch_plan_multi(b->P, b->tint, which, grid, b->stream, pa, fin)) return fail(TETRIS_E_ARG, "no planning kernel for this player count");
    HIP_TRY(hipGetLastError());
    return TETRIS_OK;
}

int tetris_action_lists_dev(tetris_batch* b, const uint8_t* d_player, int max_lists, int max_keys, int flags, int32_t* d_count,
                            uint8_t* d_lens, uint8_t* d_keys) {
    int rc = check_batch(b);
    if (rc) return rc;
    if ((rc = plan_check(b, "tetris_action_lists_dev"))) return rc;
    if (!d_count || !d_lens || !d_keys) return fail(TETRIS_E_ARG, "count/lens/keys are NULL");
    if (max_lists < 1 || max_keys < 1 || max_keys > 254) return fail(TETRIS_E_ARG, "max_lists >= 1, 1 <= max_keys <= 254");
    if (flags & ~TETRIS_LISTS_KEEP_NULL) return fail(TETRIS_E_ARG, "unknown flag");
    const int chunk = b->N < PLAN_CHUNK ? b->N : PLAN_CHUNK;
    const int KS = max_keys + 1;
    const size_t lanes = (size_t)chunk * 40;
    const size_t need = lanes + lanes * PLAN_LANE_LISTS + lanes * PLAN_LANE_LISTS * KS;
    if (!b->d_iota) {
        std::vector<int32_t> iota((size_t)b->N);
        for (int i = 0; i < b->N; i++) iota[i] = i;
        HIP_TRY(hipMalloc((void**)&b->d_iota, (size_t)b->N * 4));
        HIP_TRY(hipMemcpy(b->d_iota, iota.data(), (size_t)b->N * 4, hipMemcpyHostToDevice));
        HIP_TRY(hipMalloc((void**)&b->d_plan_status, NFLAGS * 4));
    }
    if (need > b->plan_slab_cap) {
        if (b->d_plan_slabs) { HIP_TRY(hipStreamSynchronize(b->stream)); (void)hipFree(b->d_plan_slabs); }
        b->d_plan_slabs = nullptr; b->plan_slab_cap = 0;
        HIP_TRY(hipMalloc((void**)&b->d_plan_slabs, need));
        b->plan_slab_cap = need;
    }
    if ((rc = gate_launch(b, GATE_GROUP))) return rc;
    uint8_t* s_cnt = b->d_plan_slabs;
    uint8_t* s_len = s_cnt + lanes;
    uint8_t* s_key = s_len + lanes * PLAN_LANE_LISTS;
    const Geo geo = geo_of_batch(b);
    for (int g0 = 0; g0 < b->N; g0 += chunk) {
        const int m = b->N - g0 < chunk ? b->N - g0 : chunk;
        const int32_t* d_idx = b->d_iota + g0;
        const uint8_t* pl = d_player ? d_player + g0 : nullptr;
        const dim3 grid((unsigned)(((size_t)m * 40 + 63) / 64)), block(64);
        with_value<1, 4>(b->P, [&](auto P) {
            hipLaunchKernelGGL(k_actions<P()>, grid, block, 0, b->stream, geo, m, d_idx, pl, b->H, s_cnt, s_len, s_key, PLAN_LANE_LISTS, KS, b->d_plan_status);
        });
        HIP_TRY(hipGetLastError());
        hipLaunchKernelGGL(k_plan_lists, dim3((unsigned)m), block, 0, b->stream, s_cnt, s_len, s_key, KS, g0, max_lists, max_keys,
                           (flags & TETRIS_LISTS_KEEP_NULL) ? 1 : 0, d_count, d_lens, d_keys, b->flags);
        HIP_TRY(hipGetLastError());
    }
    return TETRIS_OK;
}

int tetris_simulate_lists_dev(tetris_batch* b, const uint8_t* d_player, const int32_t* d_count, const uint8_t* d_lens, const uint8_t* d_keys,
                              int max_lists, int max_keys, int ms, int flags, uint32_t* d_cols, uint8_t* d_done, uint8_t* d_lines,
                              uint8_t* d_dead) {
    int rc = check_batch(b);
    if (rc) return rc;
    if ((rc = plan_check(b, "tetris_simulate_lists_dev"))) return rc;
    if (!d_count || !d_lens || !d_keys || !d_cols) return fail(TETRIS_E_ARG, "count/lens/keys/cols are NULL");
    if (max_lists < 1 || max_lists > 65535 || max_keys < 1 || max_keys > 255) return fail(TETRIS_E_ARG, "1 <= max_lists <= 65535, 1 <= max_keys <= 255");
    if (flags & ~TETRIS_SIM_FINALIZE) return fail(TETRIS_E_ARG, "unknown flag");
    if ((rc = gate_launch(b, GATE_GROUP))) return rc;
    PlanArgs pa = plan_args(b, d_player, d_count, d_lens, d_keys, max_lists, max_keys, ms);
    pa.cols = d_cols;
    const int fin = (flags & TETRIS_SIM_FINALIZE) ? 1 : 0;
    if (fin) { pa.a.done = d_done; pa.a.lines = d_lines; pa.a.dead = d_dead; }
    return launch_plan_kernel(b, 0, dim3((unsigned)((b->N + 63) / 64), (unsigned)max_lists), pa, fin);
}

int tetris_step_lists_dev(tetris_batch* b, const uint8_t* d_player, const int32_t* d_choice, const int32_t* d_count, const uint8_t* d_lens,
                          const uint8_t* d_keys, int max_lists, int max_keys, int ms, int flags, uint8_t* d_done, uint8_t* d_lines,
                          uint8_t* d_dead) {
    int rc = check_batch(b);
    if (rc) return rc;
    if ((rc = plan_check(b, "tetris_step_lists_dev"))) return rc;
    if (!d_choice || !d_count || !d_lens || !d_keys) return fail(TETRIS_E_ARG, "choice/count/lens/keys are NULL");
    if (max_lists < 1 || max_keys < 1 || max_keys > 255) return fail(TETRIS_E_ARG, "max_lists >= 1, 1 <= max_keys <= 255");
    if (flags & ~TETRIS_STEP_AUTO_RESET) return fail(TETRIS_E_ARG, "unknown flag");
    if ((rc = gate_launch(b, GATE_GROUP))) return rc;
    PlanArgs pa = plan_args(b, d_player, d_count, d_lens, d_keys, max_lists, max_keys, ms);
    pa.choice = d_choice;
    pa.a.done = d_done; pa.a.lines = d_lines; pa.a.dead = d_dead;
    return launch_plan_kernel(b, (flags & TETRIS_STEP_AUTO_RESET) ? 2 : 1, dim3((unsigned)((b->N + 63) / 64)), pa, 0);
}

static std::mutex g_chain_mutex;
static tetris_batch* g_chain_owner[64] = {nullptr};
static bool chain_acquire(tetris_batch* b) {
    std::lock_guard<std::mutex> lock(g_chain_mutex);
    tetris_batch*& owner = g_chain_owner[b->device & 63];
    if (owner && owner != b) return false;
    owner = b;
    return true;
}
static void chain_release(tetris_batch* b) {
    std::lock_guard<std::mutex> lock(g_chain_mutex);
    tetris_batch*& owner = g_chain_owner[b->device & 63];
    if (owner == b) owner = nullptr;
}

static bool rollout_chained(tetris_batch* b, int steps_per_launch) {
    return b->use_chain && !b->tint && !b->split && b->stream == b->own_stream &&
           (b->P == 1 || (b->P == 2 && steps_per_launch == 1 && b->use_duo)) && chain_fits(b);
}

int tetris_rollout_is_chained(tetris_batch* b, int steps_per_launch) {
    int rc = check_batch(b, false);
    if (rc) return rc;
    return rollout_chained(b, steps_per_launch) ? 1 : 0;
}

static int chain_recover(tetris_batch* b) {
    volatile uint32_t* f = b->flags;
    const RolloutCall& call = b->chain_call;
    const int lanes = chain_lanes(b);
    const int waves = (int)chain_waves(b);
    hipStream_t const home = b->own_stream;
    struct StreamGuard { tetris_batch* b; hipStream_t keep; ~StreamGuard() { b->stream = keep; } } guard{b, b->stream};
    b->stream = home;
    const size_t bytes = (size_t)waves * CHAIN_STRIDE * sizeof(uint32_t);
    if (!b->h_chain && !(b->h_chain = (uint32_t*)malloc((((size_t)b->N + 15) / 16) * sizeof(uint32_t) * CHAIN_STRIDE))) return fail(TETRIS_E_HIP, "out of host memory");
    HIP_TRY(hipMemcpyAsync(b->h_chain, b->d_chain, bytes, hipMemcpyDeviceToHost, home));
    HIP_TRY(hipStreamSynchronize(home));
    const uint32_t last = b->chain_epoch, epoch0 = call.epoch0;
    const int S = call.steps_per_launch;
    std::vector<uint32_t> stops;
    for (int w = 0; w < waves; w++) {
        const uint32_t c = b->h_chain[(size_t)w * CHAIN_STRIDE] & ~CHAIN_ABANDONED;
        if (c < epoch0 || c > last) return fail(TETRIS_E_HIP, "chained launches: an epoch word is outside the range of the call that gave up; state is invalid");
        if (c < last) stops.push_back(c);
    }
    std::sort(stops.begin(), stops.end());
    stops.erase(std::unique(stops.begin(), stops.end()), stops.end());
    const uint32_t saved_margin = b->margin;
    struct MarginGuard { tetris_batch* b; uint32_t saved; ~MarginGuard() { b->margin = saved; } } margin_guard{b, saved_margin};
    const int FUSE = 16;
    if (b->margin < (uint32_t)(2 * FUSE * 2 + 16)) b->margin = (uint32_t)(2 * FUSE * 2 + 16);
    std::vector<int32_t> idx;
    for (uint32_t c : stops) {
        idx.clear();
        for (int w = 0; w < waves; w++)
            if ((b->h_chain[(size_t)w * CHAIN_STRIDE] & ~CHAIN_ABANDONED) == c)
                for (int g = w * lanes; g < (w + 1) * lanes && g < b->N; g++) idx.push_back(g);
        unsigned long long step = call.first_step + (unsigned long long)(c - epoch0) * (unsigned long long)S;
        unsigned long long todo = (unsigned long long)(last - c) * (unsigned long long)S;
        while (todo > 0) {
            const int steps = todo < (unsigned long long)FUSE ? (int)todo : FUSE;
            Stage& s = b->recover_idx;
            int rc = s.ensure(idx.size() * 4 + 16);
            if (rc) return rc;
            memcpy(s.h, idx.data(), idx.size() * 4);
            HIP_TRY(hipMemcpyAsync(s.d, s.h, idx.size() * 4, hipMemcpyHostToDevice, home));
            KArgs a = base_args(b, (int)idx.size(), (const int32_t*)s.d);
            a.ms = call.ms; a.steps = steps; a.policy_seed = call.policy_seed; a.first_step = step;
            if ((rc = launch_game<M_ROLLOUT>(b, a))) return rc;
            HIP_TRY(hipStreamSynchronize(home));
            if ((rc = service_flags(b))) return rc;
            step += (unsigned long long)steps; todo -= (unsigned long long)steps;
        }
    }
    HIP_TRY(hipMemsetD32Async((hipDeviceptr_t)b->d_chain, (int)last, (size_t)waves * CHAIN_STRIDE, home));
    HIP_TRY(hipStreamSynchronize(home));
    f[F_CHAIN] = 0;
    b->chain_fell_back = true;
    b->use_chain = 0;
    return TETRIS_OK;
}

static KArgs rollout_args(tetris_batch* b, const RolloutCall& call, int l) {
    KArgs a = base_args(b, b->N, nullptr);
    a.ms = call.ms; a.steps = call.steps_per_launch; a.policy_seed = call.policy_seed;
    a.first_step = call.first_step + (uint64_t)l * (uint64_t)call.steps_per_launch;
    if (call.chained) { a.chain = b->d_chain; a.epoch = call.epoch0 + (uint32_t)l + 1u; a.chain_spin_limit = b->chain_spin_limit; }
    return a;
}

using Clock = std::chrono::steady_clock;
static double seconds(Clock::duration d) { return std::chrono::duration<double>(d).count(); }

static void print_stream_timing(int launches, double gate_s, Clock::time_point t_entry, Clock::time_point t_begin, Clock::time_point t_enq,
                                double ev1_us, const float* elapsed_ms) {
    const Clock::time_point now = Clock::now();
    fprintf(stderr, "[tetris timing] %d launches: host enqueue %.2f us/launch (of which gate + flags %.2f), until drained %.2f us/launch; "
            "call entry -> first enqueue %.1f us, end event seen %.1f us after the first enqueue, whole call %.1f us, between the events %.1f us\n",
            launches, seconds(t_enq - t_begin) * 1e6 / launches, gate_s * 1e6 / launches, seconds(now - t_begin) * 1e6 / launches,
            seconds(t_begin - t_entry) * 1e6, ev1_us, seconds(now - t_entry) * 1e6, elapsed_ms ? *elapsed_ms * 1e3 : 0.0);
}

static int rollout_graph(tetris_batch* b, const RolloutCall& call, float* elapsed_ms) {
    hipStream_t const home = b->stream;
    const int launches = call.launches, S = call.steps_per_launch;
    int rc = TETRIS_OK;
    HIP_TRY(hipEventRecord(b->ev0, home));
    for (int l0 = 0; l0 < launches; l0 += 128) {
        const int m = launches - l0 < 128 ? launches - l0 : 128;
        if ((rc = gate_launch(b, 1))) return rc;
        const uint32_t keep = b->margin;
        if (b->margin < (uint32_t)(2 * S * 3 * 128 + 16)) b->margin = (uint32_t)(2 * S * 3 * 128 + 16);
        hipGraph_t graph = nullptr;
        hipGraphExec_t exec = nullptr;
        HIP_TRY(hipStreamBeginCapture(home, hipStreamCaptureModeThreadLocal));
        for (int l = l0; l < l0 + m && !rc; l++) rc = launch_game<M_ROLLOUT>(b, rollout_args(b, call, l));
        b->margin = keep;
        const hipError_t ce = hipStreamEndCapture(home, &graph);
        if (rc) { if (graph) (void)hipGraphDestroy(graph); return rc; }
        HIP_TRY(ce);
        HIP_TRY(hipGraphInstantiate(&exec, graph, nullptr, nullptr, 0));
        const hipError_t le = hipGraphLaunch(exec, home);
        const hipError_t se = hipStreamSynchronize(home);
        (void)hipGraphExecDestroy(exec); (void)hipGraphDestroy(graph);
        HIP_TRY(le); HIP_TRY(se);
    }
    HIP_TRY(hipEventRecord(b->ev1, home));
    if ((rc = finish_call(b))) return rc;
    if (elapsed_ms) HIP_TRY(hipEventElapsedTime(elapsed_ms, b->ev0, b->ev1));
    return TETRIS_OK;
}

static int rollout_plain(tetris_batch* b, const RolloutCall& call, int group, Clock::time_point t_entry, float* elapsed_ms) {
    if (b->use_graph && call.steps_per_launch >= 1) return rollout_graph(b, call, elapsed_ms);
    b->last_direct = false; b->last_affine = false;
    hipStream_t const home = b->stream;
    int rc = TETRIS_OK;
    HIP_TRY(hipEventRecord(b->ev0, home));
    static const bool timing = getenv("TETRIS_TIMING") != nullptr;
    const Clock::time_point t_begin = Clock::now();
    double gate_s = 0.0;
    for (int l = 0; l < call.launches; l++) {
        const Clock::time_point t_gate = Clock::now();
        if ((rc = gate_launch(b, group))) return rc;
        if (timing) gate_s += seconds(Clock::now() - t_gate);
        if ((rc = launch_game<M_ROLLOUT>(b, rollout_args(b, call, l)))) return rc;
    }
    HIP_TRY(hipEventRecord(b->ev1, home));
    const Clock::time_point t_enq = Clock::now();
    HIP_TRY(poll_event(b->ev1, 200000));
    const double ev1_us = seconds(Clock::now() - t_begin) * 1e6;
    if ((rc = finish_call(b, true))) return rc;
    if (elapsed_ms) HIP_TRY(hipEventElapsedTime(elapsed_ms, b->ev0, b->ev1));
    if (timing) print_stream_timing(call.launches, gate_s, t_entry, t_begin, t_enq, ev1_us, elapsed_ms);
    return TETRIS_OK;
}

static hipError_t launch_chained(tetris_batch* b, const RolloutCall& call, int l, hipStream_t st) {
    const int depth = b->chain_depth;
    hipEvent_t const stop = l < call.launches - depth ? nullptr : (l == call.launches - 1 ? b->ev1 : b->chain_ev[l % depth]);
    return launch_chain_kernel(b, chain_waves(b), st, rollout_args(b, call, l), l == 0 ? b->ev0 : nullptr, stop);
}

constexpr int ENQUEUE_THREADS_MIN = 256;
static int enqueue_threaded(tetris_batch* b, const RolloutCall& call, int prefix, int group) {
    const int launches = call.launches, depth = b->chain_depth, wgroup = std::max(8, group / depth);
    b->chain_epoch = call.epoch0 + (uint32_t)launches;
    b->chain_pending = true;
    std::atomic<int> failed{0}, finished{0};
    hipError_t worker_err[CHAIN_STREAMS] = {};
    int flag_rc = TETRIS_OK;
    auto worker = [&](int k) {
        hipError_t err = hipSetDevice(b->device);
        int mine = 0, slot = 0;
        bool pending[2] = {false, false};
        hipStream_t const st = b->chain_stream[k];
        for (int l = prefix + k; l < launches && err == hipSuccess && !failed.load(std::memory_order_relaxed); l += depth) {
            if (k == 0 && !flag_rc && (flag_rc = service_flags(b))) { failed.store(1); break; }
            if (mine >= wgroup) {
                if (pending[slot] && (err = poll_event(b->worker_gate_ev[k][slot], 2000000)) != hipSuccess) break;
                if ((err = hipEventRecord(b->worker_gate_ev[k][slot], st)) != hipSuccess) break;
                pending[slot] = true; slot ^= 1; mine = 0;
            }
            mine++;
            err = launch_chained(b, call, l, st);
        }
        if (err != hipSuccess) { worker_err[k] = err; failed.store(1); }
        finished.fetch_add(1);
    };
    std::thread th[CHAIN_STREAMS];
    bool inline_k[CHAIN_STREAMS] = {};
    for (int k = 1; k < depth; k++) {
        try { th[k] = std::thread(worker, k); } catch (...) { inline_k[k] = true; }
    }
    worker(0);
    for (int k = 1; k < depth; k++) if (inline_k[k]) worker(k);
    while (finished.load() < depth) {
        if (!flag_rc && (flag_rc = service_flags(b))) failed.store(1);
        for (int spin = 0; spin < 200 && finished.load(std::memory_order_relaxed) < depth; spin++) __builtin_ia32_pause();
    }
    for (int k = 0; k < depth; k++) if (th[k].joinable()) th[k].join();
    if (flag_rc) return flag_rc;
    for (int k = 0; k < depth; k++)
        if (worker_err[k] != hipSuccess) return fail(TETRIS_E_HIP, std::string("chained launch (enqueue thread): ") + hipGetErrorString(worker_err[k]));
    return TETRIS_OK;
}

static int rollout_streams(tetris_batch* b, const RolloutCall& call, int group, bool prequeue, Clock::time_point t_entry, float* elapsed_ms) {
    b->last_direct = false; b->last_affine = false;
    hipStream_t const home = b->stream;
    const int launches = call.launches, depth = b->chain_depth;
    int rc = TETRIS_OK;
    if (prequeue) {
        ((volatile uint32_t*)b->flags)[F_GO] = 0;
        hipLaunchKernelGGL(k_blocker, dim3(1), dim3(64), 0, home, (const uint32_t*)(b->flags + F_GO), 20000000ull);
        group = 1 << 20;
    }
    struct GoGuard {
        tetris_batch* b; bool armed;
        ~GoGuard() { if (armed) ((volatile uint32_t*)b->flags)[F_GO] = 1; }
    } go_guard{b, prequeue};
    if (b->home_async || prequeue) {
        HIP_TRY(hipEventRecord(b->chain_ev[CHAIN_STREAMS], home));
        for (int k = 0; k < CHAIN_STREAMS; k++) HIP_TRY(hipStreamWaitEvent(b->chain_stream[k], b->chain_ev[CHAIN_STREAMS], 0));
    }
    static const bool timing = getenv("TETRIS_TIMING") != nullptr;
    const Clock::time_point t_begin = Clock::now();
    double gate_s = 0.0;
    const int prefix = !prequeue && launches >= ENQUEUE_THREADS_MIN ? std::min(launches, 8 * depth) : launches;
    for (int l = 0; l < prefix; l++) {
        b->stream = b->chain_stream[l % depth]; b->chain_pending = true;
        const Clock::time_point t_gate = Clock::now();
        if ((rc = gate_launch(b, group))) return rc;
        if (timing) gate_s += seconds(Clock::now() - t_gate);
        const hipError_t le = launch_chained(b, call, l, b->stream);
        if (le != hipSuccess) return fail(TETRIS_E_HIP, std::string("chained launch: ") + hipGetErrorString(le));
        b->chain_epoch++;
    }
    b->stream = home;
    if (prefix < launches && (rc = enqueue_threaded(b, call, prefix, group))) return rc;
    hipStream_t const last = b->chain_stream[(launches - 1) % depth];
    const int used = std::min(launches, depth);
    for (int k = 0; k < used; k++) HIP_TRY(hipStreamWaitEvent(home, b->chain_stream[k] != last ? b->chain_ev[k] : b->ev1, 0));
    if (prequeue) { ((volatile uint32_t*)b->flags)[F_GO] = 1; go_guard.armed = false; }
    const Clock::time_point t_enq = Clock::now();
    HIP_TRY(poll_event(b->ev1, 200000));
    for (int k = 0; k < used; k++)
        if (b->chain_stream[k] != last) HIP_TRY(poll_event(b->chain_ev[k], 200000));
    const double ev1_us = seconds(Clock::now() - t_begin) * 1e6;
    if ((rc = finish_call(b, true))) return rc;
    if (elapsed_ms) HIP_TRY(hipEventElapsedTime(elapsed_ms, b->ev0, b->ev1));
    if (timing) print_stream_timing(launches, gate_s, t_entry, t_begin, t_enq, ev1_us, elapsed_ms);
    return TETRIS_OK;
}

static int rollout_direct(tetris_batch* b, aql::Device* dev, const RolloutCall& call, int group, Clock::time_point t_entry, float* elapsed_ms) {
    static const bool timing = getenv("TETRIS_TIMING") != nullptr;
    if (b->home_async) { HIP_TRY(hipStreamSynchronize(b->stream)); }
    b->last_direct = true; b->direct_used = true;
    if (timing) fprintf(stderr, "[tetris timing] call entry -> direct dispatch %.1f us\n", seconds(Clock::now() - t_entry) * 1e6);
    aql::Queues& qs = dev->qs;
    const int launches = call.launches, depth = b->chain_depth;
    const bool affine = b->use_affine && qs.affine_ok && (b->P == 1 ? dev->chain1_affine.ok : dev->duo_affine.ok);
    b->last_affine = affine;
    const aql::Kernel& kern = affine ? (b->P == 1 ? dev->chain1_affine : dev->duo_affine) : (b->P == 1 ? dev->chain1 : dev->duo);
    uint32_t blocks = chain_waves(b);
    if (affine) blocks = (blocks + 7u) & ~7u;
    const int wgroup = std::min(aql::SLOTS / 2 - 2, std::max(8, group / depth));
    const int mid = affine ? HSA_FENCE_SCOPE_NONE : HSA_FENCE_SCOPE_AGENT, last_release = affine ? HSA_FENCE_SCOPE_SYSTEM : HSA_FENCE_SCOPE_AGENT;
    const Clock::time_point t_begin = Clock::now();
    uint64_t h_begin = 0, h_seen = 0;
    if (timing) (void)hsa_system_get_info(HSA_SYSTEM_INFO_TIMESTAMP, &h_begin);
    b->chain_epoch = call.epoch0 + (uint32_t)launches;
    aql::Pending pd;
    bool gate_pending[CHAIN_STREAMS][2] = {}, done_armed[CHAIN_STREAMS] = {};
    int mine[CHAIN_STREAMS] = {}, gate_slot[CHAIN_STREAMS] = {};
    auto drain = [&]() {
        aql::ring(qs, pd);
        bool ok = true;
        for (int k = 0; k < depth; k++) {
            if (!pd.wrote[k]) continue;
            if (!done_armed[k]) {
                hsa_signal_store_relaxed(qs.done[k], 1);
                aql::write_barrier(qs, pd, k, qs.done[k]);
                done_armed[k] = true;
                aql::ring(qs, pd);
            }
            ok = aql::wait_signal(qs.done[k]) && ok;
        }
        return ok;
    };
    struct DrainGuard { decltype(drain)& d; bool armed; ~DrainGuard() { if (armed) (void)d(); } } guard{drain, true};
    hsa_signal_t start_sig = qs.first, end_sig = qs.done[(launches - 1) % depth];
    int rc = TETRIS_OK, unflushed = 0;
    for (int l = 0; l < launches; l++) {
        const int k = l % depth;
        if ((rc = service_flags(b))) return rc;
        hsa_signal_t sig{};
        const bool first_on_queue = l < depth, last_on_queue = l >= launches - depth;
        if (last_on_queue) { hsa_signal_store_relaxed(qs.done[k], 1); sig = qs.done[k]; done_armed[k] = true; if (l == 0) start_sig = sig; }
        else if (l == 0) { hsa_signal_store_relaxed(qs.first, 1); sig = qs.first; }
        else if (mine[k] >= wgroup) {
            const int sl = gate_slot[k];
            if (gate_pending[k][sl]) { aql::ring(qs, pd); if (!aql::wait_signal(qs.gate[k][sl])) return fail(TETRIS_E_HIP, "direct dispatch: a flow-control signal never came"); }
            hsa_signal_store_relaxed(qs.gate[k][sl], 1);
            sig = qs.gate[k][sl]; gate_pending[k][sl] = true; gate_slot[k] = sl ^ 1; mine[k] = 0;
        }
        mine[k]++;
        KArgs a = rollout_args(b, call, l);
        const bool ring_wraps = qs.issued[k].load() % aql::SLOTS == 0;
        a.xcd_base = qs.xcd_base[k] + b->xcd_skew; a.xcd_slot = (uint32_t)k;
        aql::write_dispatch(qs, pd, k, kern, &a, sizeof a, blocks, first_on_queue ? HSA_FENCE_SCOPE_SYSTEM : (ring_wraps ? HSA_FENCE_SCOPE_AGENT : mid),
                            last_on_queue ? last_release : mid, sig);
        if (++unflushed >= 8 || l < 2 * depth || l == launches - 1) { aql::ring(qs, pd); unflushed = 0; }
    }
    b->chain_pending = true;
    const Clock::time_point t_enq = Clock::now();
    guard.armed = false;
    if (!drain()) return fail(TETRIS_E_HIP, "direct dispatch: a completion signal never came");
    b->chain_pending = false;
    const Clock::time_point t_seen = Clock::now();
    const double seen_us = seconds(t_seen - t_begin) * 1e6;
    if (timing) (void)hsa_system_get_info(HSA_SYSTEM_INFO_TIMESTAMP, &h_seen);
    float ms_events = 0.0f;
    hsa_amd_profiling_dispatch_time_t t0{}, t1{};
    if (hsa_amd_profiling_get_dispatch_time(dev->gpu, start_sig, &t0) == HSA_STATUS_SUCCESS &&
        hsa_amd_profiling_get_dispatch_time(dev->gpu, end_sig, &t1) == HSA_STATUS_SUCCESS && t1.end >= t0.start)
        ms_events = (float)((double)(t1.end - t0.start) * 1e3 / (double)dev->ts_freq);
    if (affine)
        for (int k = 0; k < depth; k++) {
            const uint32_t seen = ((volatile uint32_t*)b->flags)[F_XCC0 + k];
            if (seen & 0x100u) { qs.xcd_base[k] = seen & 7u; ((volatile uint32_t*)b->flags)[F_XCC0 + k] = 0; }
        }
    const bool was_misplaced = ((volatile uint32_t*)b->flags)[F_PLACE] != 0;
    if ((rc = finish_call(b, true))) return rc;
    if (affine && !was_misplaced) b->affine_failures = 0;
    if (elapsed_ms) *elapsed_ms = ms_events;
    if (timing) {
        const double tick_us = 1e6 / (double)dev->ts_freq;
        fprintf(stderr, "[tetris timing] %d launches, direct dispatch: host enqueue %.2f us/launch, last signal seen %.1f us after the first enqueue, between first start and last end %.1f us; "
                "first enqueue -> first start %.1f us, last end -> seen %.1f us, after that %.1f us\n",
                launches, seconds(t_enq - t_begin) * 1e6 / launches, seen_us, ms_events * 1e3, (double)(int64_t)(t0.start - h_begin) * tick_us,
                (double)(int64_t)(h_seen - t1.end) * tick_us, seconds(Clock::now() - t_seen) * 1e6);
    }
    return TETRIS_OK;
}

int tetris_rollout_launch(tetris_batch* b, int launches, int steps_per_launch, uint32_t policy_seed, uint64_t first_step,
                          int ms, float* elapsed_ms) {
    const Clock::time_point t_entry = Clock::now();
    int rc = check_batch(b);
    if (rc) return rc;
    if (launches < 1 || steps_per_launch < 0) return fail(TETRIS_E_ARG, "launches must be >= 1, steps_per_launch >= 0");
    if (steps_per_launch > 256) return fail(TETRIS_E_ARG, "steps_per_launch must be <= 256");
    struct MarginGuard {
        tetris_batch* b; uint32_t saved;
        ~MarginGuard() { b->margin = saved; }
    } margin_guard{b, b->margin};
    int group = steps_per_launch ? GATE_GROUP / steps_per_launch : GATE_GROUP;
    group = group < 1 ? 1 : group;
    const uint32_t need = (uint32_t)(2 * steps_per_launch * (2 * group + 2) + 16);
    if (b->margin < need) b->margin = need;
    const bool chained = rollout_chained(b, steps_per_launch) && chain_acquire(b);
    struct ChainGuard {
        tetris_batch* b; bool held; hipStream_t home;
        ~ChainGuard() {
            b->stream = home;
            if (!held) return;
            if (b->chain_pending)
                for (int k = 0; k < CHAIN_STREAMS; k++) (void)hipStreamSynchronize(b->chain_stream[k]);
            chain_release(b);
        }
    } chain_guard{b, chained, b->stream};
    RolloutCall call{0, first_step, steps_per_launch, policy_seed, ms, launches, chained};
    if (!chained) return rollout_plain(b, call, group, t_entry, elapsed_ms);
    if (b->chain_epoch + (uint32_t)launches >= CHAIN_EPOCH_MAX || b->chain_epoch + (uint32_t)launches < b->chain_epoch) {
        HIP_TRY(hipMemsetAsync(b->d_chain, 0, (((size_t)b->N + 15) / 16) * sizeof(uint32_t) * CHAIN_STRIDE, b->stream));
        b->chain_epoch = 0;
        b->home_async = true;
    }
    call.epoch0 = b->chain_epoch;
    b->chain_call = call;
    const bool prequeue = getenv("TETRIS_PREQUEUE") != nullptr && launches <= 600;
    if (!prequeue && b->direct_min > 0) {
        aql::Device* dev = aql::device_for(b->device);
        std::string why = dev->why;
        if (!(dev->ok && aql::make_queues(dev, why))) {
            b->direct_min = 0;
            if (getenv("TETRIS_TIMING")) fprintf(stderr, "[tetris] direct dispatch is off: %s\n", why.c_str());
        } else if (aql::calibrate_affine(dev), launches >= b->direct_min)
            return rollout_direct(b, dev, call, group, t_entry, elapsed_ms);
    }
    return rollout_streams(b, call, group, prequeue, t_entry, elapsed_ms);
}

int tetris_rollout_random(tetris_batch* b, int launches, int steps_per_launch, uint32_t policy_seed, uint64_t first_step,
                          int ms, uint64_t counters[4], float* elapsed_ms) {
    uint64_t before[4] = {0, 0, 0, 0}, after[4] = {0, 0, 0, 0};
    int rc;
    if (counters && (rc = tetris_rollout_totals(b, before))) return rc;
    if ((rc = tetris_rollout_launch(b, launches, steps_per_launch, policy_seed, first_step, ms, elapsed_ms))) return rc;
    if (counters) {
        if ((rc = tetris_rollout_totals(b, after))) return rc;
        for (int k = 0; k < 4; k++) counters[k] += after[k] - before[k];
    }
    return TETRIS_OK;
}

}

template <bool FEAT>
__global__ __launch_bounds__(64) void k_policy_eval(PolicyArgs pa) {
    __shared__ uint32_t s_shapes[SHAPE_WORDS];
    s_shapes[threadIdx.x] = d_shape_table.s[threadIdx.x];
    __syncthreads();
    const int i = blockIdx.x * 64 + threadIdx.x, c = blockIdx.y;
    if (i < pa.a.n) policy_eval_lane<FEAT>(pa, i, c, s_shapes);
}
// ... 154 lines not shown
```

### drl-tetris_amd/csrc/tetris_kernels.h

```cpp
#pragma once
#include "../../include/tetris_hip.h"
#include "tetris_engine.h"

namespace te {

struct KArgs {
    uint32_t* state;
    uint32_t* gstate;
    uint32_t* status;
    const uint8_t* table;
    const uint64_t* start;
    const double* combo_pow;
    uint32_t n_draws, margin;
    int H;
    int n_games;
    int n_stride;
    int n_players;
    int nw;
    int n;
    const int32_t* idx;
    const uint8_t* keys;
    const uint8_t* lens;
    int max_keys;
    const uint8_t* rot;
// ... 25 lines not shown
    uint8_t* obs_piece;
};

enum Mode { M_INIT, M_RESET, M_MAKE, M_FINISH, M_STEP_KEYS, M_STEP_RT, M_ROLLOUT, M_SPLIT_INIT, M_SPLIT_RESET,
            M_STEP_RT_AUTO,
            M_RESET_SCHED };

struct LaneCounters { unsigned long long steps, episodes, lines, sent; };

TE_HD size_t safe_slot(const int32_t* idx, int i, int n_games) {
    if (!idx) return (size_t)i;
    const uint32_t v = (uint32_t)idx[i];
    return (size_t)(v < (uint32_t)n_games ? v : (uint32_t)n_games - 1u);
}
TE_HD int safe_player_value(int v, int P) { return v < P ? v : P - 1; }
TE_HD int safe_player(const uint8_t* player, int i, int P) { return safe_player_value(player ? (int)player[i] : 0, P); }

TE_HD bool lane_active(const KArgs& a, int i) { return i < a.n && (!a.mask || a.mask[i] != 0); }

TE_HD Geo geo_of(const KArgs& a, uint32_t* state = nullptr) {
    Geo g = {state ? state : a.state, a.gstate, (size_t)a.n_games, a.n_players, a.nw, (size_t)a.n_stride};
    return g;
}

TE_HD void report_status(const KArgs& a, uint32_t st) {
    if (!st) return;
    volatile uint32_t* f = a.status;
    if (st & ST_NEED_EXTEND) f[F_EXTEND] = a.n_draws;
    if (st & ST_STREAM_EXHAUSTED) f[F_EXHAUSTED] = 1u;
    if (st & ST_FIFO_OVERFLOW) f[F_FIFO] = 1u;
    if (st & ST_BAD_ARGUMENT) f[F_BADARG] = 1u;
}

constexpr uint32_t CHAIN_ABANDONED = 0x80000000u;
constexpr uint32_t CHAIN_EPOCH_MAX = 0x7FFF0000u;
constexpr int CHAIN_STRIDE = 32;
constexpr int CHAIN_SLEEP = 1;
constexpr uint32_t CHAIN_SPIN_LIMIT = 1u << 22;

#if defined(__HIP_DEVICE_COMPILE__)
typedef __attribute__((address_space(1))) uint32_t te_gu32;
TE_HD void or_agent(uint32_t* p, uint32_t v) { (void)__hip_atomic_fetch_or(p, v, __ATOMIC_RELAXED, __HIP_MEMORY_SCOPE_AGENT); }
TE_HD void st_flag(uint32_t* p, uint32_t v) { __hip_atomic_store((te_gu32*)p, v, __ATOMIC_RELAXED, __HIP_MEMORY_SCOPE_SYSTEM); }
TE_HD uint32_t ld_flag(const uint32_t* p) { return __hip_atomic_load((const te_gu32*)p, __ATOMIC_RELAXED, __HIP_MEMORY_SCOPE_SYSTEM); }
TE_HD void st_xcd(uint32_t* p, uint32_t v) { __hip_atomic_store((te_gu32*)p, v, __ATOMIC_RELAXED, __HIP_MEMORY_SCOPE_WAVEFRONT); }
#else
TE_HD void or_agent(uint32_t* p, uint32_t v) { *p |= v; }
TE_HD void st_flag(uint32_t* p, uint32_t v) { *(volatile uint32_t*)p = v; }
TE_HD uint32_t ld_flag(const uint32_t* p) { return *(const volatile uint32_t*)p; }
TE_HD void st_xcd(uint32_t* p, uint32_t v) { *p = v; }
#endif

TE_HD uint32_t chain_poll(const KArgs& a, uint32_t wave) {
    const uint32_t want = a.epoch - 1u;
    const uint32_t* word = a.chain + (size_t)wave * CHAIN_STRIDE;
    uint32_t v = (uint32_t)wave_uniform(ld_agent(word));
    for (uint32_t polls = 1; v != want && !(v & CHAIN_ABANDONED) && polls < a.chain_spin_limit; polls++) {
        if ((polls & 255u) == 0 && wave_uniform(ld_flag(a.status + F_PLACE)) != 0) break;
#if defined(__HIP_DEVICE_COMPILE__)
        __builtin_amdgcn_s_sleep(CHAIN_SLEEP);
#endif
        v = (uint32_t)wave_uniform(ld_agent(word));
    }
    return v;
}
TE_HD void chain_give_up(const KArgs& a, uint32_t wave, bool marker) {
    if (!marker) return;
    or_agent(a.chain + (size_t)wave * CHAIN_STRIDE, CHAIN_ABANDONED);
    st_flag(a.status + F_CHAIN, 1u);
#if defined(__HIP_DEVICE_COMPILE__)
    asm volatile("s_waitcnt vmcnt(0)" ::: "memory");
#endif
}
TE_HD bool chain_wait(const KArgs& a, uint32_t wave, bool marker) {
    const uint32_t seen = chain_poll(a, wave);
    if (seen == a.epoch - 1u) return true;
    if (!(seen & CHAIN_ABANDONED)) chain_give_up(a, wave, marker);
    return false;
}

TE_HD void chain_census(const KArgs& a, bool marker) {
#if defined(__HIP_DEVICE_COMPILE__)
    if (marker) (void)__hip_atomic_fetch_add(a.chain, 1u, __ATOMIC_RELAXED, __HIP_MEMORY_SCOPE_AGENT);
    for (uint32_t spin = 0; spin < a.chain_spin_limit; spin++) {
        if (ld_agent(a.chain) >= a.epoch) return;
        __builtin_amdgcn_s_sleep(8);
    }
    if (marker) st_agent(a.chain + CHAIN_STRIDE, 1u);
#else
    (void)a; (void)marker;
#endif
}

TE_HD Ctx make_ctx(const KArgs& a, const uint32_t* shapes, bool tint = false, bool queue = true) {
    Ctx cx;
    cx.shapes = shapes;
    cx.table = a.table;
    cx.start = a.start;
    cx.combo_pow = a.combo_pow;
    cx.n_draws = a.n_draws;
    cx.margin = a.margin;
    cx.H = a.H;
    cx.floor_bits = ~0u << a.H;
    cx.tint = tint;
    cx.queue = queue;
    return cx;
}

template <int P>
TE_HD void write_outputs(const KArgs& a, int i, const Game<P>& g, int done) {
    if (a.done) a.done[i] = (uint8_t)done;
    TE_UNROLL
    for (int p = 0; p < P; p++) {
        if (a.lines) a.lines[(size_t)p * a.n + i] = (uint8_t)g.pl[p].reward;
        if (a.dead) a.dead[(size_t)p * a.n + i] = (uint8_t)g.pl[p].dead;
    }
}

template <int P>
TE_HD void make_keys(const Ctx& cx, const KArgs& a, int i, Game<P>& g) {
    if (g.round_over) return;
    TE_UNROLL
    for (int p = 0; p < P; p++) {
        Player& q = g.pl[p];
        int len = a.lens[(size_t)p * a.n + i];
        if (q.dead) len = 0;
        for (int k = 0; k < len; k++) press_key(cx, q, a.keys[((size_t)k * P + p) * a.n + i]);
    }
}

template <int P>
TE_HD void make_rt(const Ctx& cx, Game<P>& g, int player, int r, int t) {
    if (g.round_over) return;
    TE_UNROLL
    for (int p = 0; p < P; p++)
        if (p == player && !g.pl[p].dead) play_rt(cx, g.pl[p], r, t);
}

TE_HD void policy_draw(const KArgs& a, uint32_t slot, unsigned long long step, uint32_t& w0, uint32_t& w1) {
    uint32_t w[4];
    philox4x32_10(a.policy_seed, a.game_offset + slot, (uint32_t)step, (uint32_t)(step >> 32), w);
    w0 = w[0]; w1 = w[1];
}

template <int P, int MODE, bool TINT = false, int MEM = MEM_STREAM>
TE_HD void game_load(const KArgs& a, int i, Game<P>& g) {
    const size_t slot = a.idx ? (size_t)a.idx[i] : (size_t)i;
    if (MODE != M_INIT && MODE != M_SPLIT_INIT)
        load_game<P>(geo_of(a), slot, g, TINT, P > 1 || MODE == M_SPLIT_RESET, MODE == M_ROLLOUT, MEM);
    if (MODE == M_ROLLOUT) policy_draw(a, (uint32_t)slot, a.first_step, g.draw0, g.draw1);
    if (MODE == M_STEP_RT || MODE == M_STEP_RT_AUTO) { g.draw0 = a.rot[i]; g.draw1 = (uint32_t)a.trans[i] | ((a.player ? (uint32_t)a.player[i] : 0u) << 8); }
}

template <int P, int MODE, bool TINT = false, int MEM = MEM_STREAM>
TE_HD void game_run(const KArgs& a, int i, const uint32_t* shapes, Game<P>& g, LaneCounters& cnt) {
    const size_t slot = a.idx ? (size_t)a.idx[i] : (size_t)i;
    Ctx cx = make_ctx(a, shapes, TINT, P > 1 || MODE == M_SPLIT_INIT || MODE == M_SPLIT_RESET);
    if (MODE == M_INIT) init_game<P>(cx, g, (uint32_t)(a.seeds ? (uint16_t)a.seeds[i] : 0));
    if (MODE == M_SPLIT_INIT) {
        init_game<P>(cx, g, (uint32_t)(a.seeds ? (uint16_t)a.seeds[i] : 0));
        g.flags = SPLIT_ON | (a.steps ? SPLIT_SIDE : 0u);
    } else if (MODE == M_SPLIT_RESET) {
        if (P == 1) reset_split(cx, *reinterpret_cast<Game<1>*>(&g), (uint32_t)(a.seeds ? (uint16_t)a.seeds[i] : 0));
    } else if (MODE == M_RESET) {
        reset_game<P>(cx, g, (uint32_t)(a.seeds ? (uint16_t)a.seeds[i] : 0));
    } else if (MODE == M_RESET_SCHED) {
        g.episode++;
        reset_game<P>(cx, g, episode_seed(a.game_offset + (uint32_t)slot, g.episode));
    } else if (MODE == M_MAKE) {
        make_keys<P>(cx, a, i, g);
    } else if (MODE == M_FINISH) {
        TE_UNROLL
        for (int p = 0; p < P; p++) prefetch_next(cx, g.pl[p], g.seed16, g.status);
        int done = finish_game<P>(cx, g, a.ms);
        write_outputs<P>(a, i, g, done);
    } else if (MODE == M_STEP_KEYS) {
        TE_UNROLL
        for (int p = 0; p < P; p++) prefetch_next(cx, g.pl[p], g.seed16, g.status);
        make_keys<P>(cx, a, i, g);
        int done = finish_game<P>(cx, g, a.ms);
        write_outputs<P>(a, i, g, done);
    } else if (MODE == M_STEP_RT || MODE == M_STEP_RT_AUTO) {
        TE_UNROLL
        for (int p = 0; p < P; p++) prefetch_next(cx, g.pl[p], g.seed16, g.status);
        ResetPrefetch rpf;
        rpf.ok = 0; rpf.seed16 = 0; rpf.word = 0;
        if (MODE == M_STEP_RT_AUTO) prefetch_reset(cx, episode_seed(a.game_offset + (uint32_t)slot, g.episode + 1), rpf);
        make_rt<P>(cx, g, (int)(g.draw1 >> 8), (int)(g.draw0 & 3u), (int)(g.draw1 & 0xFFu));
        int done = finish_game<P>(cx, g, a.ms);
        write_outputs<P>(a, i, g, done);
        if (MODE == M_STEP_RT_AUTO && done) {
            g.episode++;
            reset_game<P>(cx, g, episode_seed(a.game_offset + (uint32_t)slot, g.episode), &rpf);
        }
    } else if (MODE == M_ROLLOUT) {
        for (int s = 0; s < a.steps; s++) {
            unsigned long long step = a.first_step + (unsigned long long)s;
            TE_UNROLL
            for (int p = 0; p < P; p++) prefetch_next(cx, g.pl[p], g.seed16, g.status);
            ResetPrefetch rpf;
            prefetch_reset(cx, episode_seed(a.game_offset + (uint32_t)slot, g.episode + 1), rpf);
            int r = (int)(g.draw0 & 3u), t = (int)(g.draw1 % 10u);
            int player = P > 1 ? (int)(step % (unsigned long long)P) : 0;
            uint32_t sent_before = 0;
            TE_UNROLL
            for (int p = 0; p < P; p++) sent_before += g.pl[p].lines_sent;
            make_rt<P>(cx, g, player, r, t);
            int done = finish_game<P>(cx, g, a.ms);
            cnt.steps++;
            g.steps++;
            uint32_t sent_after = 0;
            TE_UNROLL
            for (int p = 0; p < P; p++) {
                sent_after += g.pl[p].lines_sent;
                if (!g.pl[p].dead) { cnt.lines += (unsigned)g.pl[p].reward; g.add_lines += (unsigned)g.pl[p].reward; }
            }
            cnt.sent += (sent_after - sent_before) & 0xFFFFu;
            g.add_sent += (sent_after - sent_before) & 0xFFFFu;
            if (done) {
                cnt.episodes++;
                g.episode++;
                reset_game<P>(cx, g, episode_seed(a.game_offset + (uint32_t)slot, g.episode), &rpf);
            }
            if (s + 1 < a.steps) policy_draw(a, (uint32_t)slot, step + 1, g.draw0, g.draw1);
        }
    }
    store_game<P>(geo_of(a), slot, g, TINT, P > 1 || MODE == M_SPLIT_INIT || MODE == M_SPLIT_RESET,
                  MODE == M_ROLLOUT || MODE == M_INIT || MODE == M_SPLIT_INIT, MEM);
    report_status(a, g.status);
}

constexpr int UNDO_WORDS = 4;
constexpr uint32_t UNDO_RAN = 1u, UNDO_SIMPLE = 2u;
TE_HD Ref undo_ref(const KArgs& a, int i) { Ref r = {a.shadow, (uint32_t)i * 4u, (size_t)a.n_stride}; return r; }
TE_HD Ref undo_copy_ref(const KArgs& a, int i) { Ref r = {a.shadow + (size_t)UNDO_WORDS * a.n_stride, (uint32_t)i * 4u, (size_t)a.n_stride}; return r; }
TE_HD uint32_t pose_pack(const Player& q) {
    return (uint32_t)q.kind | ((uint32_t)q.rot << 3) | ((uint32_t)(q.x + 4) << 5) | ((uint32_t)q.y << 9) | ((uint32_t)q.next << 14);
}
TE_HD void undo_simple_settle(Player& q, uint32_t pose, uint32_t group, uint32_t draws) {
    q.kind = (int)(pose & 7u); q.rot = (int)((pose >> 3) & 3u); q.x = (int)((pose >> 5) & 15u) - 4;
    q.y = (int)((pose >> 9) & 31u); q.next = (int)((pose >> 14) & 7u);
    q.pgroup = group; q.piece_draws = draws; q.pf_ok = 0;
    q.combo_time += 200;
}

template <bool TINT>
TE_HD void split_stage_a(const KArgs& a, const Ctx& cx, int i, Game<1>& g, int side, unsigned long long step) {
    Player& q = g.pl[0];
    const uint32_t sent_before = q.lines_sent;
    int acting, r, t;
    if (a.rot) { acting = a.player ? a.player[i] : 0; r = a.rot[i] & 3; t = a.trans[i]; }
    else {
        uint32_t w[4];
        philox4x32_10(a.policy_seed, a.game_offset + (uint32_t)i, (uint32_t)step, (uint32_t)(step >> 32), w);
        r = (int)(w[0] & 3u); t = (int)(w[1] % 10u); acting = (int)(step % 2ull);
    }
    prefetch_next(cx, q, g.seed16, g.status);
    const bool plays = !g.round_over && !q.dead && acting == side;
    if (plays) play_rt(cx, q, r, t);
    const uint32_t pose = pose_pack(q), group = q.pgroup, draws = q.piece_draws, cleared = q.lines_cleared;
    const bool ran = !g.round_over && !q.dead;
    if (side == 1) {
        uint32_t full = (~0u << q.y) & ~cx.floor_bits;
        for (int c = 0; c < NCOL; c++) full &= q.col[c];
        const bool simple = ran && !full && fits_spawn_col(cx, q, shape_of(cx, q.next, spawn_rot(q.next)), 0);
        const Ref ur = undo_ref(a, i);
        word_at(ur, 0) = pose; word_at(ur, 1) = group; word_at(ur, 2) = draws;
        word_at(ur, 3) = (ran ? UNDO_RAN : 0u) | (simple ? UNDO_SIMPLE : 0u);
        if (ran && !simple) {
            const Ref cr = undo_copy_ref(a, i);
            store_player(cr.s, cr.o, cr.ws, q, TINT);
        }
        a.xout[i] = split_settle(cx, g);
        if (simple && (q.lines_cleared != cleared || q.dead)) TE_COUNT(PC_UNDO_MISPREDICT);
    } else
        a.xout[i] = split_settle(cx, g);
    if (side == 0) g.add_sent += (q.lines_sent - sent_before) & 0xFFFFu;
}

template <int STAGE, bool TINT = false>
TE_HD void split_body(const KArgs& a, int i, const uint32_t* shapes) {
    Ctx cx = make_ctx(a, shapes, TINT);
    Game<1> g;
    const int side = a.split_side;
    const bool counting = (STAGE == 2 || STAGE == 3) && a.steps;
    load_game<1>(geo_of(a), (size_t)i, g, TINT, true, counting);
    Player& q = g.pl[0];
    if (STAGE == 0) {
        split_stage_a<TINT>(a, cx, i, g, side, a.first_step);
        store_game<1>(geo_of(a), (size_t)i, g, TINT);
    } else if (STAGE == 1) {
        const uint32_t my_a = a.xw[0][i], opp_a = a.xw[1][i];
        uint32_t w;
        if (side == 0) {
            const uint32_t sent_before = q.lines_sent;
            const bool i_died = (my_a & XW_DIED) != 0;
            const int in = (!i_died && (opp_a & XW_RAN) && !(opp_a & XW_DIED)) ? xw_sent(opp_a) : 0;
            w = split_tick(cx, g, a.ms, in);
            g.add_sent += (q.lines_sent - sent_before) & 0xFFFFu;
        } else {
            const uint32_t opp_b = a.xw[2][i];
            const bool committed = !(opp_a & XW_DIED);
            if (!committed) {
                const Ref ur = undo_ref(a, i);
                const uint32_t flags = word_at(ur, 3);
                if (flags & UNDO_SIMPLE) { TE_COUNT(PC_UNDO_SIMPLE); undo_simple_settle(q, word_at(ur, 0), word_at(ur, 1), word_at(ur, 2)); }
                else if (flags & UNDO_RAN) {
                    TE_COUNT(PC_UNDO_FULL);
                    const Ref cr = undo_copy_ref(a, i);
                    load_player(cr.s, cr.o, cr.ws, q, TINT);
                }
            }
            const uint32_t sent_before = q.lines_sent;
            const int in1 = ((opp_a & XW_RAN) && !(opp_a & XW_DIED)) ? xw_sent(opp_a) : 0;
            if (!g.round_over && in1 > 0) q.incoming = q.incoming + (float)in1 / 1.0f;
            const int in2 = (opp_b & XW_DIED) ? 0 : xw_sent(opp_b);
            if (committed && (my_a & XW_RAN) && !(my_a & XW_DIED)) g.add_sent += (uint32_t)xw_sent(my_a);
            w = split_tick(cx, g, a.ms, in2);
            g.add_sent += (q.lines_sent - sent_before) & 0xFFFFu;
        }
        a.xout[i] = w;
        store_game<1>(geo_of(a), (size_t)i, g, TINT);
    } else {
        const uint32_t opp_b = a.xw[side == 0 ? 3 : 2][i];
        const int in = (side == 0 && !(opp_b & XW_DIED)) ? xw_sent(opp_b) : 0;
        const int done = split_finish(g, in, (opp_b & XW_DEAD_NOW) != 0, (opp_b & XW_ERR) != 0);
        if (a.done) a.done[i] = (uint8_t)done;
        if (a.lines) a.lines[i] = (uint8_t)q.reward;
        if (a.dead) a.dead[i] = (uint8_t)q.dead;
        if (a.steps) {
            g.steps++;
            if (!q.dead) g.add_lines += (unsigned)q.reward;
            if (done) { g.episode++; reset_split(cx, g, episode_seed(a.game_offset + (uint32_t)i, g.episode)); }
        }
        if (STAGE == 3) split_stage_a<TINT>(a, cx, i, g, side, a.first_step + 1ull);
        store_game<1>(geo_of(a), (size_t)i, g, TINT, true, counting);
    }
    report_status(a, g.status);
}

template <int P, int MODE, bool TINT = false>
TE_HD void game_body(const KArgs& a, int i, const uint32_t* shapes, LaneCounters& cnt) {
    Game<P> g;
    game_load<P, MODE, TINT>(a, i, g);
    game_run<P, MODE, TINT>(a, i, shapes, g, cnt);
}

template <int P, bool TINT = false>
TE_HD void observe_body(const Geo& geo, int i, const int32_t* idx, int H,
                        const uint32_t* shapes, tetris_record* rec, uint8_t* round_over, int8_t* last_winner) {
    size_t slot = idx ? (size_t)idx[i] : (size_t)i;
    Game<P> g;
    load_game<P>(geo, slot, g, TINT);
    if (round_over) round_over[i] = (uint8_t)g.round_over;
    if (last_winner) last_winner[i] = (int8_t)g.last_winner;
    if (!rec) return;
    TE_UNROLL
    for (int p = 0; p < P; p++) {
        const Player& q = g.pl[p];
        tetris_record* r = &rec[(size_t)i * P + p];
        uint16_t* f16 = (uint16_t*)&r->field[0][0];
        for (int y = 0; y < TETRIS_MAX_H; y++)
            for (int c = 0; c < NCOL; c += 2) {
                uint32_t lo = (y < H) ? ((q.col[c] >> y) & 1u) : 0u;
                uint32_t hi = (y < H) ? ((q.col[c + 1] >> y) & 1u) : 0u;
                if (TINT) {
                    lo *= 1u + (((q.tint[0][c] >> y) & 1u) | (((q.tint[1][c] >> y) & 1u) << 1) | (((q.tint[2][c] >> y) & 1u) << 2));
                    hi *= 1u + (((q.tint[0][c + 1] >> y) & 1u) | (((q.tint[1][c + 1] >> y) & 1u) << 1) | (((q.tint[2][c + 1] >> y) & 1u) << 2));
                }
                f16[(y * NCOL + c) >> 1] = (uint16_t)(lo | (hi << 8));
            }
        uint32_t shape = shapes[((q.kind & 7) << 2) | (q.rot & 3)];
        int val = shape_value(q.kind);
        for (int gy = 0; gy < 4; gy++) {
            uint32_t word = 0;
            for (int gx = 0; gx < 4; gx++)
// ... 241 lines not shown
```

Before: 20.97 billion.

## Add fused chained rollout kernel with precomputed row-offset tables

Introduces a k_chain_fused kernel variant (plus an affine version) for single-player chained rollouts, selected through chain_is_fused. It also generalises state load/store to take row offsets from either a stride or a precomputed byte table, so per-row address multiplies can be avoided. The per-step rollout body is factored into rollout_step so the fused kernel can reuse it. Chain capacity is now tracked separately for fused and unfused kernels, and device initialisation fails if the fused kernel symbol is missing, which adds register-pressure and occupancy risk for the new kernel.

```diff
diff --git a/drl-tetris_amd/csrc/tetris_aql.h b/drl-tetris_amd/csrc/tetris_aql.h
--- a/drl-tetris_amd/csrc/tetris_aql.h
+++ b/drl-tetris_amd/csrc/tetris_aql.h
@@ -28,7 +28,7 @@
     hsa_amd_memory_pool_t dev_pool{};
     uint64_t ts_freq = 0;
     std::vector<hsa_executable_t> exes;
-    Kernel chain1, chain1_affine, duo, duo_affine, blocker, xcc_probe;
+    Kernel chain1, chain1_affine, chain1_fused, chain1_fused_affine, duo, duo_affine, blocker, xcc_probe;
     std::vector<std::vector<char>> images;
     Queues qs;
     std::string why;
@@ -77,6 +77,8 @@
     (void)hsa_executable_symbol_get_info(s, HSA_EXECUTABLE_SYMBOL_INFO_NAME, &name[0]);
     Kernel* k = nullptr;
     if (name.rfind("_Z7k_chainILi1EEvN2te5KArgsE", 0) == 0) k = &d->chain1;
+    else if (name.rfind("_Z13k_chain_fusedILi1EEvN2te5KArgsE", 0) == 0) k = &d->chain1_fused;
+    else if (name.rfind("_Z20k_chain_fused_affineILi1EEvN2te5KArgsE", 0) == 0) k = &d->chain1_fused_affine;
     else if (name.rfind("_Z5k_duoILi6ELb1ELb0EEvN2te5KArgsE", 0) == 0) k = &d->duo;
     else if (name.rfind("_Z9k_blockerPKjy", 0) == 0) k = &d->blocker;
     else if (name.rfind("_Z14k_chain_affineILi1EEvN2te5KArgsE", 0) == 0) k = &d->chain1_affine;
@@ -170,10 +172,11 @@
         SymCtx sc{d};
         (void)hsa_executable_iterate_agent_symbols(exe, d->gpu, on_symbol, &sc);
     }
-    if (!d->chain1.ok || !d->duo.ok) return bad("the chained kernels were not found in the loaded code objects");
-    if (d->chain1.priv || d->duo.priv) return bad("the chained kernels use scratch memory");
+    if (!d->chain1.ok || !d->chain1_fused.ok || !d->duo.ok) return bad("the chained kernels were not found in the loaded code objects");
+    if (d->chain1.priv || d->chain1_fused.priv || d->duo.priv) return bad("the chained kernels use scratch memory");
     const uint32_t explicit_bytes = (uint32_t)((sizeof(KArgs) + 7) & ~(size_t)7);
-    if (d->chain1.kernarg < explicit_bytes || d->duo.kernarg < explicit_bytes || d->chain1.kernarg > 1024 || d->duo.kernarg > 1024)
+    if (d->chain1.kernarg < explicit_bytes || d->duo.kernarg < explicit_bytes || d->chain1.kernarg > 1024 || d->duo.kernarg > 1024 ||
+        d->chain1_fused.kernarg != d->chain1.kernarg)
         return bad("unexpected kernel-argument segment size");
     d->ok = true;
     return d;
diff --git a/drl-tetris_amd/csrc/tetris_engine.h b/drl-tetris_amd/csrc/tetris_engine.h
--- a/drl-tetris_amd/csrc/tetris_engine.h
+++ b/drl-tetris_amd/csrc/tetris_engine.h
@@ -43,27 +43,35 @@
     return __builtin_amdgcn_make_buffer_rsrc(const_cast<void*>(base), (short)0, -1, 0x00020000);
 }
 constexpr int TE_AUX_NT = 2, TE_AUX_SC1 = 16;
-TE_HD uint32_t ldw(const uint32_t* base, uint32_t o, size_t word_off, int mem = MEM_STREAM) {
+TE_HD uint32_t ldw_b(const uint32_t* base, uint32_t o, size_t row_bytes, int mem = MEM_STREAM) {
     const __amdgpu_buffer_rsrc_t r = te_rsrc(base);
-    if (mem == MEM_AGENT || mem == MEM_AFFINE) return __builtin_amdgcn_raw_buffer_load_b32(r, (int)o, (int)(uint32_t)(word_off * 4u), TE_AUX_SC1);
-    return __builtin_amdgcn_raw_buffer_load_b32(r, (int)o, (int)(uint32_t)(word_off * 4u), TE_AUX_NT);
-}
-TE_HD void stw(uint32_t* base, uint32_t o, size_t word_off, uint32_t v, int mem = MEM_STREAM) {
+    if (mem == MEM_AGENT || mem == MEM_AFFINE) return __builtin_amdgcn_raw_buffer_load_b32(r, (int)o, (int)(uint32_t)row_bytes, TE_AUX_SC1);
+    return __builtin_amdgcn_raw_buffer_load_b32(r, (int)o, (int)(uint32_t)row_bytes, TE_AUX_NT);
+}
+TE_HD void stw_b(uint32_t* base, uint32_t o, size_t row_bytes, uint32_t v, int mem = MEM_STREAM) {
     const __amdgpu_buffer_rsrc_t r = te_rsrc(base);
-    if (mem == MEM_AGENT) __builtin_amdgcn_raw_buffer_store_b32(v, r, (int)o, (int)(uint32_t)(word_off * 4u), TE_AUX_SC1);
-    else if (mem == MEM_AFFINE) __builtin_amdgcn_raw_buffer_store_b32(v, r, (int)o, (int)(uint32_t)(word_off * 4u), 0);
-    else __builtin_amdgcn_raw_buffer_store_b32(v, r, (int)o, (int)(uint32_t)(word_off * 4u), TE_AUX_NT);
+    if (mem == MEM_AGENT) __builtin_amdgcn_raw_buffer_store_b32(v, r, (int)o, (int)(uint32_t)row_bytes, TE_AUX_SC1);
+    else if (mem == MEM_AFFINE) __builtin_amdgcn_raw_buffer_store_b32(v, r, (int)o, (int)(uint32_t)row_bytes, 0);
+    else __builtin_amdgcn_raw_buffer_store_b32(v, r, (int)o, (int)(uint32_t)row_bytes, TE_AUX_NT);
 }
 #else
-TE_HD uint32_t ldw(const uint32_t* base, uint32_t o, size_t word_off, int mem = MEM_STREAM) {
-    const uint32_t* p = (const uint32_t*)((const char*)(base + word_off) + o);
+TE_HD uint32_t ldw_b(const uint32_t* base, uint32_t o, size_t row_bytes, int mem = MEM_STREAM) {
+    const uint32_t* p = (const uint32_t*)((const char*)base + row_bytes + o);
     return mem != MEM_STREAM ? ld_agent(p) : ld_stream(p);
 }
-TE_HD void stw(uint32_t* base, uint32_t o, size_t word_off, uint32_t v, int mem = MEM_STREAM) {
-    uint32_t* p = (uint32_t*)((char*)(base + word_off) + o);
+TE_HD void stw_b(uint32_t* base, uint32_t o, size_t row_bytes, uint32_t v, int mem = MEM_STREAM) {
+    uint32_t* p = (uint32_t*)((char*)base + row_bytes + o);
     if (mem != MEM_STREAM) st_agent(p, v); else st_stream(p, v);
 }
 #endif
+TE_HD uint32_t ldw(const uint32_t* base, uint32_t o, size_t word_off, int mem = MEM_STREAM) { return ldw_b(base, o, word_off * 4u, mem); }
+TE_HD void stw(uint32_t* base, uint32_t o, size_t word_off, uint32_t v, int mem = MEM_STREAM) { stw_b(base, o, word_off * 4u, v, mem); }
+struct RowStride { size_t ws; };
+template <int N>
+struct RowTable { uint32_t bytes[N]; };
+TE_HD size_t row_bytes(const RowStride& r, int w) { return (size_t)w * r.ws * 4u; }
+template <int N>
+TE_HD size_t row_bytes(const RowTable<N>& r, int w) { return r.bytes[w]; }
 #if defined(__HIP_DEVICE_COMPILE__)
 TE_HD void add_word(uint32_t* p, uint32_t v) { (void)__hip_atomic_fetch_add(p, v, __ATOMIC_RELAXED, __HIP_MEMORY_SCOPE_AGENT); }
 #else
@@ -178,124 +186,154 @@
     uint32_t draw0, draw1;
 };
 
-TE_HD void load_player(const uint32_t* s, uint32_t o, size_t ws, Player& q, bool tint, bool queue = true, int mem = MEM_STREAM) {
-    for (int c = 0; c < NCOL; c++) q.col[c] = ldw(s, o, (size_t)(W_COL0 + c) * ws, mem);
+template <class ROWS>
+TE_HD void load_player_rows(const uint32_t* s, uint32_t o, const ROWS& rows, Player& q, bool tint, bool queue = true, int mem = MEM_STREAM) {
+    for (int c = 0; c < NCOL; c++) q.col[c] = ldw_b(s, o, row_bytes(rows, W_COL0 + c), mem);
     if (tint)
         for (int k = 0; k < 3; k++)
-            for (int c = 0; c < NCOL; c++) q.tint[k][c] = ldw(s, o, (size_t)(W_TINT0 + 10 * k + c) * ws, mem);
-    uint32_t w = ldw(s, o, (size_t)W_PIECE * ws, mem);
+            for (int c = 0; c < NCOL; c++) q.tint[k][c] = ldw_b(s, o, row_bytes(rows, W_TINT0 + 10 * k + c), mem);
+    uint32_t w = ldw_b(s, o, row_bytes(rows, W_PIECE), mem);
     q.kind = w & 7; q.rot = (w >> 3) & 3; q.x = (int)((w >> 5) & 15) - 4; q.y = (w >> 9) & 31;
     q.next = (w >> 14) & 7; q.dead = (w >> 17) & 1; q.lock_armed = (w >> 18) & 1; q.reward = (w >> 19) & 255;
-    w = ldw(s, o, (size_t)W_MISC * ws, mem);
+    w = ldw_b(s, o, row_bytes(rows, W_MISC), mem);
     q.inc_count = w & 255; q.combo_count = (w >> 8) & 255; q.line_count = (w >> 16) & 255;
     q.qlen = (w >> 24) & 15; q.q_overflow = (w >> 28) & 3;
     if (!queue) { q.inc_count = 0; q.qlen = 0; q.q_overflow = 0; }
-    q.time_ms = (int32_t)ldw(s, o, (size_t)W_TIME * ws, mem);
-    w = ldw(s, o, (size_t)W_DROPCOMBO * ws, mem);
+    q.time_ms = (int32_t)ldw_b(s, o, row_bytes(rows, W_TIME), mem);
+    w = ldw_b(s, o, row_bytes(rows, W_DROPCOMBO), mem);
     q.drop_delay = w & 0xFFFF; q.combo_remaining = w >> 16;
-    q.drop_time = (int32_t)ldw(s, o, (size_t)W_DROP_TIME * ws, mem);
-    q.speedup_time = (int32_t)ldw(s, o, (size_t)W_SPEEDUP_TIME * ws, mem);
-    q.lock_time = (int32_t)ldw(s, o, (size_t)W_LOCK_TIME * ws, mem);
-    q.combo_start = (int32_t)ldw(s, o, (size_t)W_COMBO_START * ws, mem);
-    q.combo_time = (int32_t)ldw(s, o, (size_t)W_COMBO_TIME * ws, mem);
-    q.incoming = queue ? u2f(ldw(s, o, (size_t)W_INCOMING * ws, mem)) : 0.0f;
-    q.min_remaining = queue ? (int32_t)ldw(s, o, (size_t)W_MIN_REMAINING * ws, mem) : 1000;
-    q.piece_draws = ldw(s, o, (size_t)W_PIECE_DRAWS * ws, mem);
-    q.hole_draws = queue ? ldw(s, o, (size_t)W_HOLE_DRAWS * ws, mem) : 0u;
-    q.pgroup = ldw(s, o, (size_t)W_PIECE_GROUP * ws, mem);
-    w = ldw(s, o, (size_t)W_STATS0 * ws, mem); q.lines_sent = w & 0xFFFF; q.lines_cleared = w >> 16;
-    w = ldw(s, o, (size_t)W_STATS1 * ws, mem); q.lines_blocked = w & 0xFFFF; q.max_combo = w >> 16;
-    w = ldw(s, o, (size_t)W_STATS2 * ws, mem); q.lines_seen = w & 0xFFFF; q.garbage_cleared = w >> 16;
+    q.drop_time = (int32_t)ldw_b(s, o, row_bytes(rows, W_DROP_TIME), mem);
+    q.speedup_time = (int32_t)ldw_b(s, o, row_bytes(rows, W_SPEEDUP_TIME), mem);
+    q.lock_time = (int32_t)ldw_b(s, o, row_bytes(rows, W_LOCK_TIME), mem);
+    q.combo_start = (int32_t)ldw_b(s, o, row_bytes(rows, W_COMBO_START), mem);
+    q.combo_time = (int32_t)ldw_b(s, o, row_bytes(rows, W_COMBO_TIME), mem);
+    q.incoming = queue ? u2f(ldw_b(s, o, row_bytes(rows, W_INCOMING), mem)) : 0.0f;
+    q.min_remaining = queue ? (int32_t)ldw_b(s, o, row_bytes(rows, W_MIN_REMAINING), mem) : 1000;
+    q.piece_draws = ldw_b(s, o, row_bytes(rows, W_PIECE_DRAWS), mem);
+    q.hole_draws = queue ? ldw_b(s, o, row_bytes(rows, W_HOLE_DRAWS), mem) : 0u;
+    q.pgroup = ldw_b(s, o, row_bytes(rows, W_PIECE_GROUP), mem);
+    w = ldw_b(s, o, row_bytes(rows, W_STATS0), mem); q.lines_sent = w & 0xFFFF; q.lines_cleared = w >> 16;
+    w = ldw_b(s, o, row_bytes(rows, W_STATS1), mem); q.lines_blocked = w & 0xFFFF; q.max_combo = w >> 16;
+    w = ldw_b(s, o, row_bytes(rows, W_STATS2), mem); q.lines_seen = w & 0xFFFF; q.garbage_cleared = w >> 16;
     q.q_loaded = queue && q.qlen > 0;
     q.pf_ok = 0; q.pf_raw.lo = 0; q.pf_raw.hi = 0;
     if (queue)
         for (int i = 0; i < FIFO_CAP; i++) { q.qcount[i] = 0; q.qdelay[i] = 0; }
     if (q.q_loaded) {
         for (int i = 0; i < FIFO_CAP / 2; i++) {
-            uint32_t cw = ldw(s, o, (size_t)(W_FIFO_COUNT0 + i) * ws, mem);
+            uint32_t cw = ldw_b(s, o, row_bytes(rows, W_FIFO_COUNT0 + i), mem);
             q.qcount[2 * i] = (int16_t)(cw & 0xFFFF);
             q.qcount[2 * i + 1] = (int16_t)(cw >> 16);
         }
-        for (int i = 0; i < FIFO_CAP; i++) q.qdelay[i] = (int32_t)ldw(s, o, (size_t)(W_FIFO_DELAY0 + i) * ws, mem);
-    }
-}
-
-template <int P>
-TE_HD void load_game_words(const Ref& gr, Game<P>& g, bool counters = false, int mem = MEM_STREAM) {
-    uint32_t meta = ldw(gr.s, gr.o, (size_t)G_META * gr.ws, mem);
+        for (int i = 0; i < FIFO_CAP; i++) q.qdelay[i] = (int32_t)ldw_b(s, o, row_bytes(rows, W_FIFO_DELAY0 + i), mem);
+    }
+}
+
+TE_HD void load_player(const uint32_t* s, uint32_t o, size_t ws, Player& q, bool tint, bool queue = true, int mem = MEM_STREAM) {
+    load_player_rows(s, o, RowStride{ws}, q, tint, queue, mem);
+}
+
+template <int P, class ROWS>
+TE_HD void load_game_words_rows(const Ref& gr, const ROWS& rows, Game<P>& g, bool counters = false, int mem = MEM_STREAM) {
+    uint32_t meta = ldw_b(gr.s, gr.o, row_bytes(rows, G_META), mem);
     g.seed16 = meta & 0xFFFFu;
     g.round_over = (meta >> 16) & 1;
     g.last_winner = (int)((meta >> 17) & 0xF) - 1;
     g.flags = (meta >> 21) & 7u;
-    g.episode = ldw(gr.s, gr.o, (size_t)G_EPISODE * gr.ws, mem);
-    g.steps = counters ? ldw(gr.s, gr.o, (size_t)G_STEPS * gr.ws, mem) : 0u;
+    g.episode = ldw_b(gr.s, gr.o, row_bytes(rows, G_EPISODE), mem);
+    g.steps = counters ? ldw_b(gr.s, gr.o, row_bytes(rows, G_STEPS), mem) : 0u;
     g.add_lines = 0; g.add_sent = 0;
     g.status = 0;
 }
 
 template <int P>
-TE_HD void load_game(const Geo& geo_in, size_t slot, Game<P>& g, bool tint = false, bool queue = true, bool counters = false, int mem = MEM_STREAM) {
+TE_HD void load_game_words(const Ref& gr, Game<P>& g, bool counters = false, int mem = MEM_STREAM) {
+    load_game_words_rows<P>(gr, RowStride{gr.ws}, g, counters, mem);
+}
+
+template <int P, class ROWS, class GROWS>
+TE_HD void load_game_rows(const Geo& geo_in, size_t slot, const ROWS& rows, const GROWS& grows, Game<P>& g, bool tint = false, bool queue = true,
+                          bool counters = false, int mem = MEM_STREAM) {
     Geo geo = geo_in;
     geo.P = P;
-    load_game_words<P>(game_ref(geo, slot), g, counters, mem);
+    load_game_words_rows<P>(game_ref(geo, slot), grows, g, counters, mem);
     TE_UNROLL
     for (int p = 0; p < P; p++) {
         const Ref r = board_ref(geo, p, slot);
-        load_player(r.s, r.o, r.ws, g.pl[p], tint, queue, mem);
-    }
-}
-
-TE_HD void store_player(uint32_t* s, uint32_t o, size_t ws, const Player& q, bool tint, bool queue = true, int mem = MEM_STREAM) {
-    for (int c = 0; c < NCOL; c++) stw(s, o, (size_t)(W_COL0 + c) * ws, q.col[c], mem);
+        load_player_rows(r.s, r.o, rows, g.pl[p], tint, queue, mem);
+    }
+}
+template <int P>
+TE_HD void load_game(const Geo& geo_in, size_t slot, Game<P>& g, bool tint = false, bool queue = true, bool counters = false, int mem = MEM_STREAM) {
+    load_game_rows<P>(geo_in, slot, RowStride{(size_t)P * geo_in.stride}, RowStride{geo_in.stride}, g, tint, queue, counters, mem);
+}
+
+template <class ROWS>
+TE_HD void store_player_rows(uint32_t* s, uint32_t o, const ROWS& rows, const Player& q, bool tint, bool queue = true, int mem = MEM_STREAM) {
+    for (int c = 0; c < NCOL; c++) stw_b(s, o, row_bytes(rows, W_COL0 + c), q.col[c], mem);
     if (tint)
         for (int k = 0; k < 3; k++)
-            for (int c = 0; c < NCOL; c++) stw(s, o, (size_t)(W_TINT0 + 10 * k + c) * ws, q.tint[k][c], mem);
-    stw(s, o, (size_t)W_PIECE * ws, (uint32_t)q.kind | ((uint32_t)q.rot << 3) | ((uint32_t)(q.x + 4) << 5) | ((uint32_t)q.y << 9) |
+            for (int c = 0; c < NCOL; c++) stw_b(s, o, row_bytes(rows, W_TINT0 + 10 * k + c), q.tint[k][c], mem);
+    stw_b(s, o, row_bytes(rows, W_PIECE), (uint32_t)q.kind | ((uint32_t)q.rot << 3) | ((uint32_t)(q.x + 4) << 5) | ((uint32_t)q.y << 9) |
                               ((uint32_t)q.next << 14) | ((uint32_t)q.dead << 17) | ((uint32_t)q.lock_armed << 18) |
                               ((uint32_t)(q.reward & 255) << 19), mem);
-    stw(s, o, (size_t)W_MISC * ws, (uint32_t)(q.inc_count & 255) | ((uint32_t)(q.combo_count & 255) << 8) |
+    stw_b(s, o, row_bytes(rows, W_MISC), (uint32_t)(q.inc_count & 255) | ((uint32_t)(q.combo_count & 255) << 8) |
                              ((uint32_t)(q.line_count & 255) << 16) | ((uint32_t)q.qlen << 24) | ((uint32_t)q.q_overflow << 28), mem);
-    stw(s, o, (size_t)W_TIME * ws, (uint32_t)q.time_ms, mem);
-    stw(s, o, (size_t)W_DROPCOMBO * ws, ((uint32_t)q.drop_delay & 0xFFFF) | (q.combo_remaining << 16), mem);
-    stw(s, o, (size_t)W_DROP_TIME * ws, (uint32_t)q.drop_time, mem);
-    stw(s, o, (size_t)W_SPEEDUP_TIME * ws, (uint32_t)q.speedup_time, mem);
-    stw(s, o, (size_t)W_LOCK_TIME * ws, (uint32_t)q.lock_time, mem);
-    stw(s, o, (size_t)W_COMBO_START * ws, (uint32_t)q.combo_start, mem);
-    stw(s, o, (size_t)W_COMBO_TIME * ws, (uint32_t)q.combo_time, mem);
-    if (queue) stw(s, o, (size_t)W_INCOMING * ws, f2u(q.incoming), mem);
-    stw(s, o, (size_t)W_MIN_REMAINING * ws, (uint32_t)q.min_remaining, mem);
-    stw(s, o, (size_t)W_PIECE_DRAWS * ws, q.piece_draws, mem);
-    if (queue) stw(s, o, (size_t)W_HOLE_DRAWS * ws, q.hole_draws, mem);
-    stw(s, o, (size_t)W_PIECE_GROUP * ws, q.pgroup, mem);
-    stw(s, o, (size_t)W_STATS0 * ws, (q.lines_sent & 0xFFFF) | (q.lines_cleared << 16), mem);
-    stw(s, o, (size_t)W_STATS1 * ws, (q.lines_blocked & 0xFFFF) | (q.max_combo << 16), mem);
-    stw(s, o, (size_t)W_STATS2 * ws, (q.lines_seen & 0xFFFF) | (q.garbage_cleared << 16), mem);
+    stw_b(s, o, row_bytes(rows, W_TIME), (uint32_t)q.time_ms, mem);
+    stw_b(s, o, row_bytes(rows, W_DROPCOMBO), ((uint32_t)q.drop_delay & 0xFFFF) | (q.combo_remaining << 16), mem);
+    stw_b(s, o, row_bytes(rows, W_DROP_TIME), (uint32_t)q.drop_time, mem);
+    stw_b(s, o, row_bytes(rows, W_SPEEDUP_TIME), (uint32_t)q.speedup_time, mem);
+    stw_b(s, o, row_bytes(rows, W_LOCK_TIME), (uint32_t)q.lock_time, mem);
+    stw_b(s, o, row_bytes(rows, W_COMBO_START), (uint32_t)q.combo_start, mem);
+    stw_b(s, o, row_bytes(rows, W_COMBO_TIME), (uint32_t)q.combo_time, mem);
+    if (queue) stw_b(s, o, row_bytes(rows, W_INCOMING), f2u(q.incoming), mem);
+    stw_b(s, o, row_bytes(rows, W_MIN_REMAINING), (uint32_t)q.min_remaining, mem);
+    stw_b(s, o, row_bytes(rows, W_PIECE_DRAWS), q.piece_draws, mem);
+    if (queue) stw_b(s, o, row_bytes(rows, W_HOLE_DRAWS), q.hole_draws, mem);
+    stw_b(s, o, row_bytes(rows, W_PIECE_GROUP), q.pgroup, mem);
+    stw_b(s, o, row_bytes(rows, W_STATS0), (q.lines_sent & 0xFFFF) | (q.lines_cleared << 16), mem);
+    stw_b(s, o, row_bytes(rows, W_STATS1), (q.lines_blocked & 0xFFFF) | (q.max_combo << 16), mem);
+    stw_b(s, o, row_bytes(rows, W_STATS2), (q.lines_seen & 0xFFFF) | (q.garbage_cleared << 16), mem);
     if (queue && (q.q_loaded || q.qlen > 0)) {
         for (int i = 0; i < FIFO_CAP / 2; i++)
-            stw(s, o, (size_t)(W_FIFO_COUNT0 + i) * ws, ((uint32_t)q.qcount[2 * i] & 0xFFFF) | ((uint32_t)q.qcount[2 * i + 1] << 16), mem);
-        for (int i = 0; i < FIFO_CAP; i++) stw(s, o, (size_t)(W_FIFO_DELAY0 + i) * ws, (uint32_t)q.qdelay[i], mem);
-    }
+            stw_b(s, o, row_bytes(rows, W_FIFO_COUNT0 + i), ((uint32_t)q.qcount[2 * i] & 0xFFFF) | ((uint32_t)q.qcount[2 * i + 1] << 16), mem);
+        for (int i = 0; i < FIFO_CAP; i++) stw_b(s, o, row_bytes(rows, W_FIFO_DELAY0 + i), (uint32_t)q.qdelay[i], mem);
+    }
+}
+
+TE_HD void store_player(uint32_t* s, uint32_t o, size_t ws, const Player& q, bool tint, bool queue = true, int mem = MEM_STREAM) {
+    store_player_rows(s, o, RowStride{ws}, q, tint, queue, mem);
+}
+
+template <int P, class ROWS>
+TE_HD void store_game_words_rows(const Ref& gr, const ROWS& rows, const Game<P>& g, bool counters = false, int mem = MEM_STREAM) {
+    stw_b(gr.s, gr.o, row_bytes(rows, G_META), g.seed16 | ((uint32_t)g.round_over << 16) | ((uint32_t)(g.last_winner + 1) << 17) | (g.flags << 21), mem);
+    stw_b(gr.s, gr.o, row_bytes(rows, G_EPISODE), g.episode, mem);
+    if (counters) stw_b(gr.s, gr.o, row_bytes(rows, G_STEPS), g.steps, mem);
+    if (g.add_lines) add_word((uint32_t*)((char*)gr.s + row_bytes(rows, G_LINES) + gr.o), g.add_lines);
+    if (g.add_sent) add_word((uint32_t*)((char*)gr.s + row_bytes(rows, G_SENT) + gr.o), g.add_sent);
 }
 
 template <int P>
 TE_HD void store_game_words(const Ref& gr, const Game<P>& g, bool counters = false, int mem = MEM_STREAM) {
-    stw(gr.s, gr.o, (size_t)G_META * gr.ws, g.seed16 | ((uint32_t)g.round_over << 16) | ((uint32_t)(g.last_winner + 1) << 17) | (g.flags << 21), mem);
-    stw(gr.s, gr.o, (size_t)G_EPISODE * gr.ws, g.episode, mem);
-    if (counters) stw(gr.s, gr.o, (size_t)G_STEPS * gr.ws, g.steps, mem);
-    if (g.add_lines) add_word(&word_at(gr, G_LINES), g.add_lines);
-    if (g.add_sent) add_word(&word_at(gr, G_SENT), g.add_sent);
-}
-
-template <int P>
-TE_HD void store_game(const Geo& geo_in, size_t slot, const Game<P>& g, bool tint = false, bool queue = true, bool counters = false, int mem = MEM_STREAM) {
+    store_game_words_rows<P>(gr, RowStride{gr.ws}, g, counters, mem);
+}
+
+template <int P, class ROWS, class GROWS>
+TE_HD void store_game_rows(const Geo& geo_in, size_t slot, const ROWS& rows, const GROWS& grows, const Game<P>& g, bool tint = false, bool queue = true,
+                           bool counters = false, int mem = MEM_STREAM) {
     Geo geo = geo_in;
     geo.P = P;
-    store_game_words<P>(game_ref(geo, slot), g, counters, mem);
+    store_game_words_rows<P>(game_ref(geo, slot), grows, g, counters, mem);
     TE_UNROLL
     for (int p = 0; p < P; p++) {
         const Ref r = board_ref(geo, p, slot);
-        store_player(r.s, r.o, r.ws, g.pl[p], tint, queue, mem);
-    }
+        store_player_rows(r.s, r.o, rows, g.pl[p], tint, queue, mem);
+    }
+}
+template <int P>
+TE_HD void store_game(const Geo& geo_in, size_t slot, const Game<P>& g, bool tint = false, bool queue = true, bool counters = false, int mem = MEM_STREAM) {
+    store_game_rows<P>(geo_in, slot, RowStride{(size_t)P * geo_in.stride}, RowStride{geo_in.stride}, g, tint, queue, counters, mem);
 }
 
 
diff --git a/drl-tetris_amd/csrc/tetris_hip.hip b/drl-tetris_amd/csrc/tetris_hip.hip
--- a/drl-tetris_amd/csrc/tetris_hip.hip
+++ b/drl-tetris_amd/csrc/tetris_hip.hip
@@ -24,7 +24,7 @@
 
 constexpr int CHAIN_LANES = 64;
 constexpr int CHAIN_STREAMS = 3;
-template <int P, bool AFFINE>
+template <int P, bool AFFINE, bool FUSED>
 __device__ __forceinline__ void chain_body(const KArgs& a) {
     __shared__ __attribute__((aligned(16))) uint32_t s_shapes[SHAPE_WORDS];
     const int lane = threadIdx.x;
@@ -53,14 +53,42 @@
     const uint32_t d0 = g.draw0, d1 = g.draw1;
     int stride = a.n_stride;
     asm volatile("" : "+s"(stride));
+    RowTable<NWORDS> rows = {};
+    RowTable<NGWORDS> grows = {};
+    if (!FUSED) {
+        TE_UNROLL
+        for (int w = 0; w < NWORDS; w++)
+            if (P > 1 || (w < NWORDS_HOT && w != W_INCOMING && w != W_HOLE_DRAWS)) {
+                uint32_t bytes = (uint32_t)(w * P) * (uint32_t)stride * 4u;
+                asm volatile("" : "+s"(bytes));
+                rows.bytes[w] = bytes;
+            }
+        TE_UNROLL
+        for (int w = 0; w < NGWORDS; w++) {
+            uint32_t bytes = (uint32_t)w * (uint32_t)stride * 4u;
+            asm volatile("" : "+s"(bytes));
+            grows.bytes[w] = bytes;
+        }
+    }
     const uint32_t seen = chain_poll(a, (uint32_t)wave);
     if (seen == a.epoch - 1u) {
         Geo geo = geo_of(a);
         geo.stride = (size_t)stride;
-        if (active) { load_game<P>(geo, (size_t)i, g, false, P > 1, true, CMEM); g.draw0 = d0; g.draw1 = d1; }
+        if (active) {
+            if (FUSED) load_game<P>(geo, (size_t)i, g, false, P > 1, true, CMEM);
+            else load_game_rows<P>(geo, (size_t)i, rows, grows, g, false, P > 1, true, CMEM);
+            g.draw0 = d0; g.draw1 = d1;
+        }
         s_shapes[lane] = shape_word;
         __builtin_amdgcn_wave_barrier();
-        if (active) game_run<P, M_ROLLOUT, false, CMEM>(a, i, s_shapes, g, cnt);
+        if (FUSED) {
+            if (active) game_run<P, M_ROLLOUT, false, CMEM>(a, i, s_shapes, g, cnt);
+        } else if (active) {
+            const Ctx cx = make_ctx(a, s_shapes, false, P > 1);
+            rollout_step<P>(cx, a, (size_t)i, a.first_step, g, cnt);
+            store_game_rows<P>(geo, (size_t)i, rows, grows, g, false, P > 1, true, CMEM);
+            report_status(a, g.status);
+        }
         asm volatile("s_waitcnt vmcnt(0)" ::: "memory");
         if (lane == 0) {
             if (AFFINE) st_xcd(a.chain + (size_t)wave * CHAIN_STRIDE, a.epoch);
@@ -72,10 +100,15 @@
     report_xcc();
 }
 template <int P>
-__global__ __launch_bounds__(64) void k_chain(KArgs a) { chain_body<P, false>(a); }
+__global__ __launch_bounds__(64) void k_chain(KArgs a) { chain_body<P, false, false>(a); }
 template <int P>
-__global__ __launch_bounds__(64) void k_chain_affine(KArgs a) { chain_body<P, true>(a); }
+__global__ __launch_bounds__(64) void k_chain_affine(KArgs a) { chain_body<P, true, false>(a); }
+template <int P>
+__global__ __launch_bounds__(64) void k_chain_fused(KArgs a) { chain_body<P, false, true>(a); }
+template <int P>
+__global__ __launch_bounds__(64) void k_chain_fused_affine(KArgs a) { chain_body<P, true, true>(a); }
 template __global__ void k_chain_affine<1>(KArgs);
+template __global__ void k_chain_fused_affine<1>(KArgs);
 extern "C" __global__ void tetris_k_xcc_probe(uint32_t* out) {
     if (threadIdx.x == 0) {
         uint32_t xcc;
@@ -831,7 +864,7 @@
     uint32_t chain_epoch = 0;
     int use_chain = 1;
     int use_graph = 0;
-    long long chain_capacity = -1;
+    long long chain_capacity[2] = {-1, -1};
     int chain_depth = 0;
     bool chain_pending = false;
     uint32_t chain_spin_limit = CHAIN_SPIN_LIMIT;
@@ -901,17 +934,19 @@
 static int chain_lanes(const tetris_batch* b) { return b->P == 1 ? CHAIN_LANES : 32; }
 static uint32_t chain_waves(const tetris_batch* b) { return (uint32_t)((b->N + chain_lanes(b) - 1) / chain_lanes(b)); }
 
-static const void* chain_kernel(tetris_batch* b, long long* waves) {
+static bool chain_is_fused(const tetris_batch* b, int steps_per_launch) { return b->P == 1 && steps_per_launch != 1; }
+static const void* chain_kernel(tetris_batch* b, bool fused, long long* waves) {
     *waves = chain_waves(b);
-    return b->P == 1 ? (const void*)k_chain<1> : (const void*)k_duo<M_ROLLOUT, true>;
-}
-static hipError_t launch_chain_kernel(tetris_batch* b, uint32_t blocks, hipStream_t st, const KArgs& a, hipEvent_t start = nullptr,
+    return b->P == 1 ? (fused ? (const void*)k_chain_fused<1> : (const void*)k_chain<1>) : (const void*)k_duo<M_ROLLOUT, true>;
+}
+static hipError_t launch_chain_kernel(tetris_batch* b, bool fused, uint32_t blocks, hipStream_t st, const KArgs& a, hipEvent_t start = nullptr,
                                       hipEvent_t stop = nullptr) {
-    if (b->P == 1) hipExtLaunchKernelGGL((k_chain<1>), dim3(blocks), dim3(64), 0, st, start, stop, 0, a);
+    if (b->P == 1 && fused) hipExtLaunchKernelGGL((k_chain_fused<1>), dim3(blocks), dim3(64), 0, st, start, stop, 0, a);
+    else if (b->P == 1) hipExtLaunchKernelGGL((k_chain<1>), dim3(blocks), dim3(64), 0, st, start, stop, 0, a);
     else hipExtLaunchKernelGGL((k_duo<M_ROLLOUT, true>), dim3(blocks), dim3(64), 0, st, start, stop, 0, a);
     return hipGetLastError();
 }
-static bool chain_census_ok(tetris_batch* b, long long waves) {
+static bool chain_census_ok(tetris_batch* b, bool fused, long long waves) {
     uint32_t* d = nullptr;
     if (hipMalloc((void**)&d, 2 * CHAIN_STRIDE * sizeof(uint32_t)) != hipSuccess) return false;
     bool ok = false;
@@ -920,7 +955,7 @@
     memset(&a, 0, sizeof a);
     a.steps = -1; a.chain = d; a.epoch = (uint32_t)waves; a.chain_spin_limit = 4000;
     if (hipMemsetAsync(d, 0, 2 * CHAIN_STRIDE * sizeof(uint32_t), b->own_stream) == hipSuccess) {
-        if (launch_chain_kernel(b, (uint32_t)waves, b->own_stream, a) == hipSuccess && hipMemcpyAsync(&h[0], d, 4, hipMemcpyDeviceToHost, b->own_stream) == hipSuccess &&
+        if (launch_chain_kernel(b, fused, (uint32_t)waves, b->own_stream, a) == hipSuccess && hipMemcpyAsync(&h[0], d, 4, hipMemcpyDeviceToHost, b->own_stream) == hipSuccess &&
             hipMemcpyAsync(&h[1], d + CHAIN_STRIDE, 4, hipMemcpyDeviceToHost, b->own_stream) == hipSuccess &&
             hipStreamSynchronize(b->own_stream) == hipSuccess)
             ok = h[0] == (uint32_t)waves && h[1] == 0;
@@ -929,24 +964,25 @@
     return ok;
 }
 
-static bool chain_fits(tetris_batch* b) {
+static bool chain_fits(tetris_batch* b, bool fused) {
     long long waves = 0;
-    const void* fn = chain_kernel(b, &waves);
+    const void* fn = chain_kernel(b, fused, &waves);
+    long long& capacity = b->chain_capacity[fused ? 1 : 0];
     static const int cap = [] { const char* e = getenv("TETRIS_CHAIN_DEPTH"); const int v = e ? atoi(e) : CHAIN_STREAMS; return v < 1 ? 1 : (v > CHAIN_STREAMS ? CHAIN_STREAMS : v); }();
-    if (b->chain_capacity < 0) {
+    if (capacity < 0) {
         int per_cu = 0, cus = 0;
         if (hipOccupancyMaxActiveBlocksPerMultiprocessor(&per_cu, fn, 64, 0) != hipSuccess) per_cu = 0;
         if (hipDeviceGetAttribute(&cus, hipDeviceAttributeMultiprocessorCount, b->device) != hipSuccess) cus = 0;
-        b->chain_capacity = per_cu > 1 ? (long long)(per_cu - 1) * cus : 0;
+        capacity = per_cu > 1 ? (long long)(per_cu - 1) * cus : 0;
         const long long full = (long long)per_cu * cus;
         int want = 0;
         for (int d = cap; d >= 2 && !want; d--)
             if (d * waves <= full) want = d;
-        if (want && want * waves > b->chain_capacity && b->stream == b->own_stream && chain_census_ok(b, want * waves)) b->chain_capacity = want * waves;
+        if (want && want * waves > capacity && b->stream == b->own_stream && chain_census_ok(b, fused, want * waves)) capacity = want * waves;
     }
     b->chain_depth = 0;
     for (int d = cap; d >= 1 && !b->chain_depth; d--)
-        if (d * waves <= b->chain_capacity) b->chain_depth = d;
+        if (d * waves <= capacity) b->chain_depth = d;
     return b->chain_depth >= (cap == 1 ? 1 : 2);
 }
 
@@ -1991,7 +2027,7 @@
 
 static bool rollout_chained(tetris_batch* b, int steps_per_launch) {
     return b->use_chain && !b->tint && !b->split && b->stream == b->own_stream &&
-           (b->P == 1 || (b->P == 2 && steps_per_launch == 1 && b->use_duo)) && chain_fits(b);
+           (b->P == 1 || (b->P == 2 && steps_per_launch == 1 && b->use_duo)) && chain_fits(b, chain_is_fused(b, steps_per_launch));
 }
 
 int tetris_rollout_is_chained(tetris_batch* b, int steps_per_launch) {
@@ -2135,7 +2171,7 @@
 static hipError_t launch_chained(tetris_batch* b, const RolloutCall& call, int l, hipStream_t st) {
     const int depth = b->chain_depth;
     hipEvent_t const stop = l < call.launches - depth ? nullptr : (l == call.launches - 1 ? b->ev1 : b->chain_ev[l % depth]);
-    return launch_chain_kernel(b, chain_waves(b), st, rollout_args(b, call, l), l == 0 ? b->ev0 : nullptr, stop);
+    return launch_chain_kernel(b, chain_is_fused(b, call.steps_per_launch), chain_waves(b), st, rollout_args(b, call, l), l == 0 ? b->ev0 : nullptr, stop);
 }
 
 constexpr int ENQUEUE_THREADS_MIN = 256;
@@ -2237,9 +2273,11 @@
     if (timing) fprintf(stderr, "[tetris timing] call entry -> direct dispatch %.1f us\n", seconds(Clock::now() - t_entry) * 1e6);
     aql::Queues& qs = dev->qs;
     const int launches = call.launches, depth = b->chain_depth;
-    const bool affine = b->use_affine && qs.affine_ok && (b->P == 1 ? dev->chain1_affine.ok : dev->duo_affine.ok);
+    const bool fused = chain_is_fused(b, call.steps_per_launch);
+    const aql::Kernel& one = fused ? dev->chain1_fused : dev->chain1, & one_affine = fused ? dev->chain1_fused_affine : dev->chain1_affine;
+    const bool affine = b->use_affine && qs.affine_ok && (b->P == 1 ? one_affine.ok && !one_affine.priv : dev->duo_affine.ok);
     b->last_affine = affine;
-    const aql::Kernel& kern = affine ? (b->P == 1 ? dev->chain1_affine : dev->duo_affine) : (b->P == 1 ? dev->chain1 : dev->duo);
+    const aql::Kernel& kern = affine ? (b->P == 1 ? one_affine : dev->duo_affine) : (b->P == 1 ? one : dev->duo);
     uint32_t blocks = chain_waves(b);
     if (affine) blocks = (blocks + 7u) & ~7u;
     const int wgroup = std::min(aql::SLOTS / 2 - 2, std::max(8, group / depth));
diff --git a/drl-tetris_amd/csrc/tetris_kernels.h b/drl-tetris_amd/csrc/tetris_kernels.h
--- a/drl-tetris_amd/csrc/tetris_kernels.h
+++ b/drl-tetris_amd/csrc/tetris_kernels.h
@@ -201,6 +201,36 @@
     if (MODE == M_STEP_RT || MODE == M_STEP_RT_AUTO) { g.draw0 = a.rot[i]; g.draw1 = (uint32_t)a.trans[i] | ((a.player ? (uint32_t)a.player[i] : 0u) << 8); }
 }
 
+template <int P>
+TE_HD void rollout_step(const Ctx& cx, const KArgs& a, size_t slot, unsigned long long step, Game<P>& g, LaneCounters& cnt) {
+    TE_UNROLL
+    for (int p = 0; p < P; p++) prefetch_next(cx, g.pl[p], g.seed16, g.status);
+    ResetPrefetch rpf;
+    prefetch_reset(cx, episode_seed(a.game_offset + (uint32_t)slot, g.episode + 1), rpf);
+    int r = (int)(g.draw0 & 3u), t = (int)(g.draw1 % 10u);
+    int player = P > 1 ? (int)(step % (unsigned long long)P) : 0;
+    uint32_t sent_before = 0;
+    TE_UNROLL
+    for (int p = 0; p < P; p++) sent_before += g.pl[p].lines_sent;
+    make_rt<P>(cx, g, player, r, t);
+    int done = finish_game<P>(cx, g, a.ms);
+    cnt.steps++;
+    g.steps++;
+    uint32_t sent_after = 0;
+    TE_UNROLL
+    for (int p = 0; p < P; p++) {
+        sent_after += g.pl[p].lines_sent;
+        if (!g.pl[p].dead) { cnt.lines += (unsigned)g.pl[p].reward; g.add_lines += (unsigned)g.pl[p].reward; }
+    }
+    cnt.sent += (sent_after - sent_before) & 0xFFFFu;
+    g.add_sent += (sent_after - sent_before) & 0xFFFFu;
+    if (done) {
+        cnt.episodes++;
+        g.episode++;
+        reset_game<P>(cx, g, episode_seed(a.game_offset + (uint32_t)slot, g.episode), &rpf);
+    }
+}
+
 template <int P, int MODE, bool TINT = false, int MEM = MEM_STREAM>
 TE_HD void game_run(const KArgs& a, int i, const uint32_t* shapes, Game<P>& g, LaneCounters& cnt) {
     const size_t slot = a.idx ? (size_t)a.idx[i] : (size_t)i;
@@ -245,32 +275,7 @@
     } else if (MODE == M_ROLLOUT) {
         for (int s = 0; s < a.steps; s++) {
             unsigned long long step = a.first_step + (unsigned long long)s;
-            TE_UNROLL
-            for (int p = 0; p < P; p++) prefetch_next(cx, g.pl[p], g.seed16, g.status);
-            ResetPrefetch rpf;
-            prefetch_reset(cx, episode_seed(a.game_offset + (uint32_t)slot, g.episode + 1), rpf);
-            int r = (int)(g.draw0 & 3u), t = (int)(g.draw1 % 10u);
-            int player = P > 1 ? (int)(step % (unsigned long long)P) : 0;
-            uint32_t sent_before = 0;
-            TE_UNROLL
-            for (int p = 0; p < P; p++) sent_before += g.pl[p].lines_sent;
-            make_rt<P>(cx, g, player, r, t);
-            int done = finish_game<P>(cx, g, a.ms);
-            cnt.steps++;
-            g.steps++;
-            uint32_t sent_after = 0;
-            TE_UNROLL
-            for (int p = 0; p < P; p++) {
-                sent_after += g.pl[p].lines_sent;
-                if (!g.pl[p].dead) { cnt.lines += (unsigned)g.pl[p].reward; g.add_lines += (unsigned)g.pl[p].reward; }
-            }
-            cnt.sent += (sent_after - sent_before) & 0xFFFFu;
-            g.add_sent += (sent_after - sent_before) & 0xFFFFu;
-            if (done) {
-                cnt.episodes++;
-                g.episode++;
-                reset_game<P>(cx, g, episode_seed(a.game_offset + (uint32_t)slot, g.episode), &rpf);
-            }
+            rollout_step<P>(cx, a, slot, step, g, cnt);
             if (s + 1 < a.steps) policy_draw(a, (uint32_t)slot, step + 1, g.draw0, g.draw1);
         }
     }
```

New measurement: 22.41 billion, median of 6. 1.07x the previous value.
